# gpcv-liujin/Deep3D_Aerial

Hardware: AMD Instinct MI355X
Metric: cost-volume Mvoxels/s (5v x 384D) (higher is better)
Workload: dtype f32; 1 GPU; config 2: fused homography-warp + variance, 5 views x 384 planes, features 32x688x464 fp32 (2752x1856 image at 1/4 res), one reference view per step per GPU

## Files before the change

deep3d_aerial_amd/_lib.py:

```python
import ctypes
import os
import subprocess

_HERE = os.path.dirname(os.path.abspath(__file__))
CSRC = os.path.join(_HERE, "csrc")
SO_PATH = os.environ.get("D3D_LIBRARY") or os.path.join(CSRC, "libdeep3d_planesweep.so")
HEADER = os.path.join(os.path.dirname(_HERE), "include", "deep3d_planesweep.h")

ABI_VERSION = 11

_vp = ctypes.c_void_p
_i = ctypes.c_int
_i64 = ctypes.c_int64
_f = ctypes.c_float
_d = ctypes.c_double
_sz = ctypes.c_size_t

SIGNATURES = {
    "d3d_version": [],
    "d3d_last_error": ([], ctypes.c_char_p),
    "d3d_compose_projections": [_vp, _i, _vp, _vp],
    "d3d_debug_force_path": [_i],
    "d3d_debug_dispatch_counts": [_vp, _i],
    "d3d_build_flags": ([], ctypes.c_char_p),
    "d3d_h16_format": ([], ctypes.c_char_p),
    "d3d_compose_projections_f64": [_vp, _i, _vp, _vp],
    "d3d_homo_warp_f64coord": [_vp, _vp, _vp, _i, _i, _i, _i, _i, _vp, _vp],
    "d3d_sweep_workspace_bytes": ([_i, _i, _i, _i, _i, _i], _sz),
    "d3d_sweep_workspace_bytes_for": ([_i, _i, _i, _i, _i, _i, _i], _sz),
    "d3d_homo_warp": [_vp, _vp, _vp, _i, _i, _i, _i, _i, _vp, _vp, _sz, _vp],
    "d3d_variance_volume": [ctypes.POINTER(_vp), _vp, _vp, _i, _i, _i, _i, _i, _i, _vp, _vp, _sz, _vp],
    "d3d_variance_volume_planes": [ctypes.POINTER(_vp), _vp, _vp, _i, _i, _i, _i, _i, _i, _vp, _vp, _sz, _vp],
    "d3d_variance_volume_f16": [ctypes.POINTER(_vp), _vp, _vp, _i, _i, _i, _i, _i, _i, _vp, _vp, _sz, _vp],
    "d3d_variance_volume_cl_h16": [ctypes.POINTER(_vp), _vp, _vp, _i, _i, _i, _i, _i, _i, _vp, _vp, _sz, _vp],
    "d3d_variance_volume_cl8_h16": [ctypes.POINTER(_vp), _vp, _vp, _i, _i, _i, _i, _i, _i, _vp, _vp, _sz, _vp],
    "d3d_pair_corr_mean": [_vp, _vp, _vp, _vp, _i, _i, _i, _i, _i, _vp, _vp, _sz, _vp],
    "d3d_weighted_corr": [ctypes.POINTER(_vp), _vp, _vp, _vp, _i, _i, _i, _i, _i, _i, _i, _vp, _vp, _sz, _vp],
    "d3d_softargmin_conf4": [_vp, _vp, _i, _i, _i, _i, _vp, _vp, _vp],
    "d3d_online_regress_update": [_vp, _vp, _i, _i, _i, _i, _vp, _vp, _vp, _vp],
    "d3d_online_regress_finalize": [_vp, _vp, _vp, _i64, _vp, _vp, _vp],
    "d3d_depth_range_samples": [_vp, _i, _i, _f, _i, _i, _vp, _vp],
    "d3d_resize_bilinear": [_vp, _i, _i, _i, _i, _i, _vp, _vp],
    "d3d_conv3d_k3": [_vp, _vp, _vp, _vp, _vp, _i, _i, _i, _i, _i, _i, _i, _vp, _vp],
    "d3d_conv3d_k3_co8": [_vp, _vp, _vp, _vp, _vp, _i, _i, _i, _i, _i, _vp, _vp],
    "d3d_conv3d_k3_c8_h16": [_vp, _vp, _vp, _vp, _vp, _i, _i, _i, _i, _i, _vp, _vp],
    "d3d_conv3d_k3_zs_h16": [_vp, _vp, _vp, _vp, _vp, _i, _i, _i, _i, _i, _i, _vp, _vp],
    "d3d_conv3d_k3_zs_bf16x3": [_vp, _vp, _vp, _vp, _vp, _i, _i, _i, _i, _i, _i, _vp, _vp],
    "d3d_conv3d_k3_c1_bf16x3": [_vp, _vp, _vp, _vp, _vp, _i, _i, _i, _i, _i, _vp, _vp],
    "d3d_convtranspose3d_k3s2_zs_h16": [_vp, _vp, _vp, _vp, _vp, _i, _i, _i, _i, _i, _i, _vp, _vp],
    "d3d_convtranspose3d_k3s2_zs_bf16x3": [_vp, _vp, _vp, _vp, _vp, _i, _i, _i, _i, _i, _i, _vp, _vp],
    "d3d_conv2d_k3_zs_h16": [_vp, _i, _vp, _i, _vp, _vp, _vp, _vp, _vp, _i, _i, _i, _i, _i, _i, _vp, _vp],
    "d3d_conv2d_k3_zs_f32": [_vp, _i, _vp, _i, _vp, _vp, _vp, _vp, _vp, _i, _i, _i, _i, _i, _i, _vp, _vp],
    "d3d_conv2d_k3_zs_bf16x3": [_vp, _i, _vp, _i, _vp, _vp, _vp, _vp, _vp, _i, _i, _i, _i, _i, _i, _vp, _vp],
    "d3d_avgpool2d_4_8": [_vp, _i, _i, _i, _vp, _vp, _vp],
    "d3d_conv3x3_bias_border": [_vp, _vp, _i, _i, _i, _vp],
    "d3d_conv2d_k1_f32": [_vp, _vp, _vp, _vp, _vp, _i, _i, _i, _i, _i, _vp, _vp],
    "d3d_conv1x1_context": [_vp, _i, _vp, _vp, _i, _i, _vp, _i, _i, _i, _i, _i, _vp, _vp],
    "d3d_conv2d_k3s2_zs_h16": [_vp, _vp, _vp, _vp, _vp, _i, _i, _i, _i, _i, _i, _vp, _vp],
    "d3d_conv2d_k3s2_zs_h16_batched": [_vp, _vp, _vp, _vp, _i, _i, _i, _i, _i, _i, _i64, _i64, _vp, _vp],
    "d3d_conv2d_k3_wide_h16": [_vp, _i, _vp, _i, _vp, _vp, _vp, _vp, _i, _i, _i, _i, _vp, _vp],
    "d3d_slice_head_regress_h16": [_vp, _vp, _vp, _i, _vp, _i, _i, _i, _i, _vp, _vp, _vp, _vp],
    "d3d_gru_cell_fused_h16": [_vp, _i, _i, _i, _i, _vp, _i, _i, _i, _vp, _vp, _vp, _vp, _vp, _vp, _vp],
    "d3d_gru_cell_fused_cl8_h16": [_vp, _i, _vp, _i, _i, _i, _vp, _vp, _vp, _vp, _vp, _vp, _vp],
    "d3d_weighted_corr_cl8_h16": [ctypes.POINTER(_vp), _vp, _vp, _vp, _i, _i, _i, _i, _i, _i, _vp, _vp, _sz, _vp],
    "d3d_convtranspose2d_k3s2_zs_h16": [_vp, _vp, _vp, _vp, _vp, _i, _i, _i, _i, _i, _i, _vp, _vp],
    "d3d_conv2d_k3s2_zs_bf16x3": [_vp, _vp, _vp, _vp, _vp, _i, _i, _i, _i, _i, _i, _vp, _vp],
    "d3d_convtranspose2d_k3s2_zs_bf16x3": [_vp, _vp, _vp, _vp, _vp, _i, _i, _i, _i, _i, _i, _vp, _vp],
    "d3d_convtranspose2d_k4s2_zs_bf16x3": [_vp, _vp, _vp, _vp, _vp, _i, _i, _i, _i, _i, _i, _vp, _vp],
    "d3d_conv2d_k5s2_zs_bf16x3": [_vp, _vp, _vp, _vp, _vp, _i, _i, _i, _i, _i, _i, _vp, _vp],
    "d3d_conv2d_k3s2_zs_f32": [_vp, _vp, _vp, _vp, _vp, _i, _i, _i, _i, _i, _i, _vp, _vp],
    "d3d_convtranspose2d_k3s2_zs_f32": [_vp, _vp, _vp, _vp, _vp, _i, _i, _i, _i, _i, _i, _vp, _vp],
    "d3d_conv3d_k3_cl_h16": [_vp, _i, _vp, _vp, _vp, _vp, _i, _i, _i, _i, _i, _i, _vp, _i, _vp],
    "d3d_conv3d_k3_c1_cl_h16": [_vp, _i, _vp, _vp, _vp, _vp, _i, _i, _i, _i, _i, _vp, _vp],
    "d3d_conv3d_k3s2_cl_h16": [_vp, _vp, _vp, _vp, _vp, _i, _i, _i, _i, _i, _i, _vp, _vp],
    "d3d_convtranspose3d_k3s2_cl_h16": [_vp, _vp, _vp, _vp, _vp, _i, _i, _i, _i, _i, _i, _vp, _i, _vp],
    "d3d_conv2d_k3_zs_h16_gn": [_vp, _i, _vp, _i, _vp, _vp, _i, _i, _i, _vp, _vp, _i, _vp],
    "d3d_conv2d_k3_wide_h16_gn": [_vp, _i, _vp, _i, _vp, _vp, _i, _i, _i, _vp, _vp, _i, _vp],
    "d3d_convtranspose2d_k3s2_wide_h16": [_vp, _vp, _vp, _vp, _vp, _i, _i, _i, _i, _i, _vp, _vp],
    "d3d_conv2d_k3_pair3_bf16x3": [_vp, _vp, _vp, _vp, _i, _vp, _vp, _vp, _i, _i, _i, _i, _vp, _vp],
    "d3d_slice_tail_regress_h16": [_vp, _vp, _vp, _vp, _vp, _vp, _vp, _i, _i, _i, _i, _vp, _vp, _vp, _vp],
    "d3d_slice_tail_regress_same_h16": [_vp, _vp, _vp, _vp, _i, _vp, _vp, _vp, _i, _i, _i, _i, _vp, _vp, _vp, _vp],
    "d3d_conv3d_k3s2_zs_bf16x3": [_vp, _vp, _vp, _vp, _vp, _i, _i, _i, _i, _i, _i, _vp, _vp],
    "d3d_convtranspose3d_prob_cl_h16": [_vp, _vp, _vp, _vp, _vp, _i, _vp, _vp, _i, _i, _i, _vp, _vp],
    "d3d_volume_planar_to_cl_h16": [_vp, _i, _sz, _vp, _vp],
    "d3d_volume_cl_h16_to_planar": [_vp, _i, _sz, _vp, _vp],
    "d3d_convtranspose3d_k3s2_co8": [_vp, _vp, _vp, _vp, _vp, _i, _i, _i, _i, _i, _vp, _vp],
    "d3d_convtranspose3d_k3s2": [_vp, _vp, _vp, _vp, _vp, _i, _i, _i, _i, _i, _i, _vp, _vp],
    "d3d_conv1x1_upskip": [_vp, _i, _vp, _vp, _vp, _i, _i, _i, _vp, _vp],
    "d3d_conv2d_k3_stream": [_vp, _i, _vp, _i, _vp, _vp, _vp, _vp, _vp, _i, _i, _i, _i, _i, _vp, _vp],
    "d3d_conv2d_k3": [_vp, _i, _vp, _i, _vp, _vp, _vp, _vp, _i, _i, _i, _i, _i, _vp, _vp],
    "d3d_convtranspose2d_k3s2": [_vp, _vp, _vp, _vp, _vp, _i, _i, _i, _i, _i, _i, _vp, _vp],
    "d3d_conv_gemm_f32": [_vp, _i, _vp, _i, _vp, _i, _vp, _vp, _vp, _i, _i, _i, _i, _i, _i, _i, _i, _i, _i, _i, _i, _i,
                          _i, _i, _i, _i, _i, ctypes.c_char_p, _vp, _vp],
    "d3d_conv_fold_f32": [_vp, _i, _vp, _i, _vp, _i, _i, _vp, _vp, _vp, _i, _i, _vp, _i, _i, _i, _i, _i, _i, _i, _i,
                          ctypes.POINTER(ctypes.c_int), _i, ctypes.c_char_p, _vp, _vp],
    "d3d_conv_fold_h16": [_vp, _i, _vp, _i, _vp, _i, _i, _vp, _vp, _vp, _i, _i, _vp, _i, _i, _i, _i, _i, _i, _i, _i,
                           ctypes.POINTER(ctypes.c_int), _i, ctypes.c_char_p, _vp, _vp],
    "d3d_gru_gates": [_vp, _vp, _i, _i64, _vp, _vp, _vp],
    "d3d_gru_update": [_vp, _vp, _vp, _i64, _vp, _vp],
    "d3d_groupnorm_stats": [_vp, _i64, _i, _vp, _vp],
    "d3d_gru_gates_gn": [_vp, _vp, _vp, _vp, _vp, _vp, _vp, _vp, _i, _i64, ctypes.c_float, _i, _vp, _vp, _vp],
    "d3d_gru_update_gn": [_vp, _vp, _vp, _vp, _vp, _vp, _i, _i64, ctypes.c_float, _i, _vp, _vp],
    "d3d_gru_reset_gn": [_vp, _vp, _vp, _vp, _vp, _i, _i64, ctypes.c_float, _i, _vp, _vp],
    "d3d_gru_update_gates_gn": [_vp, _vp, _vp, _vp, _vp, _vp, _vp, _vp, _vp, _i, _i64, ctypes.c_float, _i, _vp, _vp],
    "d3d_gru2_cell_gn_h16": [_vp, _i, _vp, _i, _i, _i, _vp, _vp, _vp, _vp, _vp, _vp, _vp, _vp, _vp, _vp, ctypes.c_float, _i, _vp, _vp, _vp, _vp, _vp, _vp, _vp],
    "d3d_softargmin_conf4_var": [_vp, _vp, _i, _i, _i, _i, ctypes.c_float, _vp, _vp, _vp, _vp],
    "d3d_uncertainty_samples": [_vp, _vp, _i, _i, _i, _vp, _vp],
    "d3d_pair_softmax_max": [_vp, _vp, _i, _i, _i, _i, _vp, _vp, _vp],
    "d3d_consistency_check": [_vp, _vp, _vp, _vp, _vp, ctypes.POINTER(ctypes.c_double), _i, _i, _i, _i, ctypes.c_double,
                              _f, _f, _f, _vp, _vp, _vp, _vp, _vp, _vp],
    "d3d_fusion_ref_init": [_vp, _vp, ctypes.POINTER(ctypes.c_double), _i, _i, _vp, _vp, _vp, _vp, _vp],
    "d3d_fusion_accumulate": [_vp, _vp, _vp, _vp, _vp, ctypes.POINTER(ctypes.c_double), _i, _i, _i, _i,
                              ctypes.c_double, _f, _f, _f, _i, _vp, _vp, _vp, _vp, _vp, _vp],
    "d3d_fusion_finalize": [_vp, _vp, _vp, _i, _i, _i, _vp, _vp, _vp],
    "d3d_fusion_points_scratch_bytes": ([_i, _i], _sz),
    "d3d_fusion_mark_points": [_vp, _vp, _i, _i, _i, ctypes.POINTER(ctypes.c_double), _vp, _vp, _vp, _vp],
    "d3d_fusion_gather_points": [_vp, _vp, ctypes.POINTER(_vp), _i, _vp, _vp, _i, _i, _vp, _vp, _vp, _vp, _vp, _vp, _vp],
    "d3d_flip_rows": [ctypes.POINTER(_vp), _i, _i, _i, _vp, _vp],
    "d3d_center_image_u8": [_vp, _i, _i, _i, _i, _i, _i, _i, _i, _vp, _vp, _vp],
    "d3d_normals_from_depth": [_vp, ctypes.POINTER(_f), _i, _i, _i, _i, _vp, _vp, _vp],
    "d3d_dsm_scratch_bytes": ([ctypes.c_longlong, _i, _i, _i], _sz),
    "d3d_dsm_from_points": [_vp, ctypes.c_longlong, _d, _d, _d, _d, _d, _d, _i, _i, _i, _d, _i, _vp, _sz, _vp, _vp, _vp],
    "d3d_dsm_fill_moving_average": [_vp, _vp, _i, _i, _i, _vp],
    "d3d_dsm_mesh_scratch_bytes": ([ctypes.c_longlong, _i, _i], _sz),
    "d3d_dsm_from_mesh": [_vp, ctypes.c_longlong, _vp, ctypes.c_longlong, _d, _d, _d, _d, _d, _d, _i, _i, _vp, _sz, _vp, _vp],
    "d3d_ortho_scratch_bytes": ([_i, _i, _i], _sz),
    "d3d_ortho_select": [_vp, _d, _d, _d, _d, _i, _i, _vp, _i, _d, _vp, _sz, _vp, _vp],
    "d3d_ortho_colorize": [_vp, _d, _d, _d, _d, _i, _i, _vp, _vp, _i, _vp, _vp, _vp],
    "d3d_mesh_scan_scratch_bytes": ([ctypes.c_longlong], _sz),
    "d3d_mesh_mark": [_vp, _vp, _i, _i, _d, _vp, _vp],
    "d3d_mesh_bricks": [_vp, _vp, _vp, _sz, _vp, _vp, _vp, _vp],
    "d3d_mesh_integrate": [_vp, _vp, _i, _vp, _i, _d, _d, _vp, _vp, _vp],
    "d3d_mesh_count": [_vp, _vp, _vp, _i, _vp, _vp, _i, _vp, _sz, _vp, _vp, _vp, _vp, _vp],
    "d3d_mesh_emit": [_vp, _vp, _vp, _i, _vp, _vp, _i, _vp, _vp, _vp, _vp, _vp, _vp, _vp],
    "d3d_mesh_compact": [_vp, ctypes.c_longlong, _vp, ctypes.c_longlong, _vp, _vp, _sz, _vp, _vp, _vp, _vp],
    "d3d_mesh_adjacency_scratch_bytes": ([ctypes.c_longlong, ctypes.c_longlong], _sz),
    "d3d_mesh_adjacency": [_vp, ctypes.c_longlong, ctypes.c_longlong, _vp, _sz, _vp, _vp, _vp, _vp],
    "d3d_mesh_components": [_vp, ctypes.c_longlong, ctypes.c_longlong, _vp, _vp, ctypes.POINTER(_i), _vp],
    "d3d_mesh_stats_scratch_bytes": ([ctypes.c_longlong], _sz),
    "d3d_mesh_component_stats": [_vp, ctypes.c_longlong, _vp, ctypes.c_longlong, _vp, _vp, _sz, _vp, _vp, _vp, _vp, _vp, _vp],
    "d3d_mesh_filter_scratch_bytes": ([ctypes.c_longlong], _sz),
    "d3d_mesh_filter": [_vp, ctypes.c_longlong, ctypes.c_longlong, _vp, _vp, _vp, _vp, ctypes.c_longlong, _d, _vp, _sz, _vp, _vp, _vp, _vp],
    "d3d_mesh_smooth": [_vp, ctypes.c_longlong, _vp, _vp, _vp, _f, _i, _vp, _vp, _vp],
    "d3d_mesh_decimate_incidence_scratch_bytes": ([ctypes.c_longlong, ctypes.c_longlong], _sz),
    "d3d_mesh_decimate_incidence": [_vp, ctypes.c_longlong, ctypes.c_longlong, _vp, _sz, _vp, _vp, _vp],
    "d3d_mesh_decimate_quadrics": [_vp, ctypes.c_longlong, _vp, ctypes.c_longlong, _vp, _vp, _vp, _vp],
    "d3d_mesh_decimate_edges_scratch_bytes": ([ctypes.c_longlong], _sz),
    "d3d_mesh_decimate_edges": [_vp, _vp, ctypes.c_longlong, _vp, _sz, ctypes.c_longlong, _vp, _vp, _vp],
    "d3d_mesh_decimate_candidates": [_vp, ctypes.c_longlong, _vp, ctypes.c_longlong, _vp, _vp, _vp, _vp, _vp, _vp, _vp, _vp, ctypes.c_longlong, _vp, _vp, _vp, _vp],
    "d3d_mesh_decimate_select_scratch_bytes": ([], _sz),
    "d3d_mesh_decimate_select": [_vp, ctypes.c_longlong, ctypes.c_longlong, _vp, _sz, _vp, _vp],
    "d3d_mesh_decimate_claim": [_vp, _vp, ctypes.c_longlong, _vp, _vp, _vp, ctypes.c_longlong, _vp, _vp, _vp, _vp],
    "d3d_mesh_decimate_apply": [_vp, ctypes.c_longlong, _vp, _vp, _vp, _vp, _vp, _vp, _vp, ctypes.c_longlong, _vp, _vp, _vp, _vp, _vp, _vp, _vp],
    "d3d_mesh_decimate_faces_scratch_bytes": ([ctypes.c_longlong], _sz),
    "d3d_mesh_decimate_faces": [_vp, ctypes.c_longlong, ctypes.c_longlong, _vp, _vp, _sz, _vp, _vp, _vp, _vp],
    "d3d_mesh_holes_scratch_bytes": ([ctypes.c_longlong], _sz),
    "d3d_mesh_boundary": [_vp, ctypes.c_longlong, ctypes.c_longlong, _vp, _vp, _vp, _vp, _vp, _vp, _vp, _vp],
    "d3d_mesh_boundary_loops": [_vp, ctypes.c_longlong, ctypes.c_longlong, _vp, _vp, _vp, _vp, _vp, _vp, _vp, ctypes.POINTER(_i), _vp],
    "d3d_mesh_holes_plan": [_vp, ctypes.c_longlong, _vp, ctypes.c_longlong, _vp, _vp, _vp, _vp, _vp, _i, _vp, _sz, _vp, _vp, _vp, _vp, _vp, _vp,
                            _vp, _vp],
    "d3d_mesh_holes_emit": [_vp, ctypes.c_longlong, _vp, ctypes.c_longlong, _vp, _vp, _vp, _vp, _vp, _vp, _vp, ctypes.c_longlong,
                            ctypes.c_longlong, _vp, _vp, _vp],
    "d3d_texture_scratch_bytes": ([ctypes.c_longlong, _i], _sz),
    "d3d_texture_select": [_vp, ctypes.c_longlong, _vp, ctypes.c_longlong, _vp, _i, _d, _vp, _sz, _vp, _vp],
    "d3d_texture_edges": [_vp, ctypes.c_longlong, ctypes.c_longlong, _vp, _vp, _vp],
    "d3d_texture_charts": [_vp, _vp, ctypes.c_longlong, _vp, ctypes.c_longlong, _vp, _sz, _vp, _vp, _vp, _vp, ctypes.POINTER(_i), _vp],
    "d3d_texture_rects": [_vp, ctypes.c_longlong, _vp, ctypes.c_longlong, _vp, _vp, ctypes.c_longlong, _vp, _i, _i, _vp, _vp],
    "d3d_texture_fill": [_vp, ctypes.c_longlong, _vp, ctypes.c_longlong, _vp, _i, _vp, _i, _i, _vp, _vp],
    "d3d_texture_empty": [_vp, ctypes.c_longlong, ctypes.c_uint, _vp],
    "d3d_texture_texcoords": [_vp, ctypes.c_longlong, _vp, ctypes.c_longlong, _vp, _vp, _vp, ctypes.c_longlong, _vp, _i, _vp, _i, _i, _vp,
                              _vp, _vp],
}


class LibraryMissing(RuntimeError):
    pass


def build(verbose=False):
    cmd = ["make", "-C", CSRC, "-j4", "libdeep3d_planesweep.so"]
    res = subprocess.run(cmd, stdout=subprocess.PIPE, stderr=subprocess.STDOUT, text=True)
    if verbose or res.returncode != 0:
        print(res.stdout)
    if res.returncode != 0:
        raise RuntimeError("building libdeep3d_planesweep.so failed")
    return SO_PATH


_lib = None


def load():
    global _lib
    if _lib is not None:
        return _lib
    if not os.path.exists(SO_PATH):
        raise LibraryMissing(
            "%s not found -- build it with `python -c 'import __graft_entry__ as g; g.build()'` "
            "or `make -C deep3d_aerial_amd/csrc`. There is no CPU fallback." % SO_PATH)
    lib = ctypes.CDLL(SO_PATH)
    for name, sig in SIGNATURES.items():
        try:
            fn = getattr(lib, name)
        except AttributeError as e:
            raise LibraryMissing("symbol %s missing from %s" % (name, SO_PATH)) from e
        fn.argtypes, fn.restype = sig if isinstance(sig, tuple) else (sig, ctypes.c_int)
    if lib.d3d_version() != ABI_VERSION:
        raise LibraryMissing("ABI version mismatch: library %d, binding %d" % (lib.d3d_version(), ABI_VERSION))
    _lib = lib
    return lib


ERR_INVALID_ARG, ERR_UNSUPPORTED, ERR_HIP = -1, -2, -3


def h16_format():
    return load().d3d_h16_format().decode("ascii")


def code_objects(path=None):
    import struct

    data = open(path or SO_PATH, "rb").read()
    magic = b"__CLANG_OFFLOAD_BUNDLE__"
    pos = data.find(magic)
    while pos >= 0:
        n = struct.unpack_from("<Q", data, pos + 24)[0]
        q = pos + 32
        for _ in range(n):
            off, size, tl = struct.unpack_from("<QQQ", data, q)
            triple = data[q + 24:q + 24 + tl]
            q += 24 + tl
            if b"amdgcn" not in triple or size == 0:
                continue
            elf = data[pos + off:pos + off + size]
            if elf[:4] == b"\x7fELF":
                yield elf
        pos = data.find(magic, pos + len(magic))


def kernel_code_sha256(symbol_prefix, path=None):
    import hashlib
    import struct

    found = []
    for elf in code_objects(path):
        shoff, = struct.unpack_from("<Q", elf, 0x28)
        shentsize, shnum = struct.unpack_from("<HH", elf, 0x3A)
        secs = [struct.unpack_from("<IIQQQQIIQQ", elf, shoff + i * shentsize) for i in range(shnum)]
        for sh in secs:
            if sh[1] != 2:
                continue
            strtab = secs[sh[6]]
            for k in range(sh[5] // sh[9]):
                st_name, st_info, _, st_shndx, st_value, st_size = struct.unpack_from("<IBBHQQ", elf, sh[4] + k * sh[9])
                if (st_info & 0xF) != 2 or st_size == 0 or st_shndx >= len(secs):
                    continue
                end = elf.index(b"\0", strtab[4] + st_name)
                if elf[strtab[4] + st_name:end].decode("ascii", "replace").startswith(symbol_prefix):
                    sec = secs[st_shndx]
                    o = sec[4] + (st_value - sec[3])
                    found.append(hashlib.sha256(elf[o:o + st_size]).hexdigest())
    return found[0] if len(found) == 1 else None


def check(rc, what):
    if rc != 0:
        msg = load().d3d_last_error().decode("utf-8", "replace")
        kind = {-1: "invalid argument", -2: "unsupported", -3: "HIP error"}.get(rc, "error %d" % rc)
        raise RuntimeError("%s failed (%s): %s" % (what, kind, msg))
```

deep3d_aerial_amd/csrc/planesweep.hip:

```cpp
#include <hip/hip_fp16.h>

#include "common.h"

#include <array>
#include <atomic>
#include <cstring>
#include <mutex>
#include <unordered_map>

namespace d3d {

static thread_local char g_err[512] = "";

void set_error(const char* fmt, ...) {
    va_list ap;
    va_start(ap, fmt);
    vsnprintf(g_err, sizeof(g_err), fmt, ap);
    va_end(ap);
}

int hip_status(hipError_t e, const char* what) {
    if (e == hipSuccess) return D3D_OK;
    set_error("%s: %s", what, hipGetErrorString(e));
    return D3D_ERR_HIP;
}

int ensure_dynamic_lds(const void* kernel, int bytes) {
    constexpr int MAXDEV = 16;
    static std::mutex mu;
    static std::unordered_map<const void*, std::array<int, MAXDEV>> granted;
    int dev = 0;
    if (hipGetDevice(&dev) != hipSuccess) dev = -1;
    if (dev >= 0 && dev < MAXDEV) {
        std::lock_guard<std::mutex> lock(mu);
        auto it = granted.find(kernel);
        if (it != granted.end() && it->second[dev] >= bytes) return D3D_OK;
    }
    const int rc = hip_status(hipFuncSetAttribute(kernel, hipFuncAttributeMaxDynamicSharedMemorySize, bytes),
                              "hipFuncSetAttribute(MaxDynamicSharedMemorySize)");
    if (rc == D3D_OK && dev >= 0 && dev < MAXDEV) {
        std::lock_guard<std::mutex> lock(mu);
        auto& slot = granted[kernel];
        if (slot[dev] < bytes) slot[dev] = bytes;
    }
    return rc;
}

int launch_tiled(int mode, const struct SweepParams& p, hipStream_t stream);
int launch_window(int mode, const struct SweepParams& p, hipStream_t stream, bool forced);
size_t tiled_workspace_bytes(int n_src, int C, int D, int h, int w, int elem_bytes);
size_t window_workspace_bytes(int n_src, int C, int D, int h, int w, int elem_bytes);
const char* tiled_build_flags();
const char* window_build_flags();
const char* gru_build_flags();

}

#include "sweep_params.h"

namespace d3d {

__global__ void compose_kernel(const float* __restrict__ proj44, int n_views, float* __restrict__ out34) {
    int i = blockIdx.x * blockDim.x + threadIdx.x + 1;
    if (i >= n_views) return;
    double m[16], inv[16];
    for (int k = 0; k < 16; ++k) m[k] = (double)proj44[k];
    inv[0] = m[5] * m[10] * m[15] - m[5] * m[11] * m[14] - m[9] * m[6] * m[15] + m[9] * m[7] * m[14] +
             m[13] * m[6] * m[11] - m[13] * m[7] * m[10];
    inv[4] = -m[4] * m[10] * m[15] + m[4] * m[11] * m[14] + m[8] * m[6] * m[15] - m[8] * m[7] * m[14] -
             m[12] * m[6] * m[11] + m[12] * m[7] * m[10];
    inv[8] = m[4] * m[9] * m[15] - m[4] * m[11] * m[13] - m[8] * m[5] * m[15] + m[8] * m[7] * m[13] +
             m[12] * m[5] * m[11] - m[12] * m[7] * m[9];
    inv[12] = -m[4] * m[9] * m[14] + m[4] * m[10] * m[13] + m[8] * m[5] * m[14] - m[8] * m[6] * m[13] -
              m[12] * m[5] * m[10] + m[12] * m[6] * m[9];
    inv[1] = -m[1] * m[10] * m[15] + m[1] * m[11] * m[14] + m[9] * m[2] * m[15] - m[9] * m[3] * m[14] -
             m[13] * m[2] * m[11] + m[13] * m[3] * m[10];
    inv[5] = m[0] * m[10] * m[15] - m[0] * m[11] * m[14] - m[8] * m[2] * m[15] + m[8] * m[3] * m[14] +
             m[12] * m[2] * m[11] - m[12] * m[3] * m[10];
    inv[9] = -m[0] * m[9] * m[15] + m[0] * m[11] * m[13] + m[8] * m[1] * m[15] - m[8] * m[3] * m[13] -
             m[12] * m[1] * m[11] + m[12] * m[3] * m[9];
    inv[13] = m[0] * m[9] * m[14] - m[0] * m[10] * m[13] - m[8] * m[1] * m[14] + m[8] * m[2] * m[13] +
              m[12] * m[1] * m[10] - m[12] * m[2] * m[9];
    inv[2] = m[1] * m[6] * m[15] - m[1] * m[7] * m[14] - m[5] * m[2] * m[15] + m[5] * m[3] * m[14] +
             m[13] * m[2] * m[7] - m[13] * m[3] * m[6];
    inv[6] = -m[0] * m[6] * m[15] + m[0] * m[7] * m[14] + m[4] * m[2] * m[15] - m[4] * m[3] * m[14] -
             m[12] * m[2] * m[7] + m[12] * m[3] * m[6];
    inv[10] = m[0] * m[5] * m[15] - m[0] * m[7] * m[13] - m[4] * m[1] * m[15] + m[4] * m[3] * m[13] +
              m[12] * m[1] * m[7] - m[12] * m[3] * m[5];
    inv[14] = -m[0] * m[5] * m[14] + m[0] * m[6] * m[13] + m[4] * m[1] * m[14] - m[4] * m[2] * m[13] -
              m[12] * m[1] * m[6] + m[12] * m[2] * m[5];
    inv[3] = -m[1] * m[6] * m[11] + m[1] * m[7] * m[10] + m[5] * m[2] * m[11] - m[5] * m[3] * m[10] -
             m[9] * m[2] * m[7] + m[9] * m[3] * m[6];
    inv[7] = m[0] * m[6] * m[11] - m[0] * m[7] * m[10] - m[4] * m[2] * m[11] + m[4] * m[3] * m[10] +
             m[8] * m[2] * m[7] - m[8] * m[3] * m[6];
    inv[11] = -m[0] * m[5] * m[11] + m[0] * m[7] * m[9] + m[4] * m[1] * m[11] - m[4] * m[3] * m[9] -
              m[8] * m[1] * m[7] + m[8] * m[3] * m[5];
    inv[15] = m[0] * m[5] * m[10] - m[0] * m[6] * m[9] - m[4] * m[1] * m[10] + m[4] * m[2] * m[9] +
              m[8] * m[1] * m[6] - m[8] * m[2] * m[5];
    double det = m[0] * inv[0] + m[1] * inv[4] + m[2] * inv[8] + m[3] * inv[12];
    double idet = 1.0 / det;
    const float* s = proj44 + 16 * i;
    for (int r = 0; r < 3; ++r)
        for (int c = 0; c < 4; ++c) {
            double acc = 0.0;
            for (int k = 0; k < 4; ++k) acc += (double)s[r * 4 + k] * (inv[k * 4 + c] * idet);
            out34[(i - 1) * 12 + r * 4 + c] = (float)acc;
        }
}

struct TapD {
    int off;
    int dx, dyw;
    float nw, ne, sw, se;
};

__device__ __forceinline__ TapD make_tap_direct(float u, float v, int h, int w) {
    TapD t;
    float fu = floorf(u), fv = floorf(v);
    int x0 = (int)fu, y0 = (int)fv;
    float ax = u - fu, ay = v - fv;
    float bx = (fu + 1.0f) - u, by = (fv + 1.0f) - v;
    bool vx0 = (x0 >= 0) && (x0 < w), vx1 = (x0 >= -1) && (x0 < w - 1);
    bool vy0 = (y0 >= 0) && (y0 < h), vy1 = (y0 >= -1) && (y0 < h - 1);
    t.nw = (vx0 && vy0) ? bx * by : 0.0f;
    t.ne = (vx1 && vy0) ? ax * by : 0.0f;
    t.sw = (vx0 && vy1) ? bx * ay : 0.0f;
    t.se = (vx1 && vy1) ? ax * ay : 0.0f;
    int x0c = min(max(x0, 0), w - 1), x1c = min(max(x0 + 1, 0), w - 1);
    int y0c = min(max(y0, 0), h - 1), y1c = min(max(y0 + 1, 0), h - 1);
    t.off = y0c * w + x0c;
    t.dx = x1c - x0c;
    t.dyw = (y1c - y0c) * w;
    return t;
}

__device__ __forceinline__ float ldf(const float* p) { return *p; }
__device__ __forceinline__ float ldf(const __half* p) { return __half2float(*p); }
__device__ __forceinline__ void stf(float* p, float v) { *p = v; }
__device__ __forceinline__ void stf(__half* p, float v) {
    *p = __float2half_rn(sat_f16(v));
}

template <typename T>
__device__ __forceinline__ float gather4(const T* __restrict__ f, const TapD& t) {
    const T* q = f + t.off;
    float acc = ldf(q) * t.nw;
    acc = fmaf(ldf(q + t.dx), t.ne, acc);
    acc = fmaf(ldf(q + t.dyw), t.sw, acc);
    acc = fmaf(ldf(q + t.dyw + t.dx), t.se, acc);
    return acc;
}

template <int MODE, int CC, typename T = float>
__global__ __launch_bounds__(256) void sweep_direct_kernel(SweepParams p) {
    const int x = blockIdx.x * 64 + (threadIdx.x & 63);
    const int y = blockIdx.y * 4 + (threadIdx.x >> 6);
    if (x >= p.w || y >= p.h) return;
    const int h = p.h, w = p.w, C = p.C, D = p.D;
    const size_t plane = (size_t)h * w;
    const size_t pix = (size_t)y * w + x;
    const float xf = (float)x, yf = (float)y;
    const int d0 = blockIdx.z * p.d_chunk;
    const int d1 = min(d0 + p.d_chunk, D);
    const float invV = 1.0f / (float)(p.n_src + 1);

    for (int d = d0; d < d1; ++d) {
        const float dv = p.depth_mode == D3D_DEPTH_PER_PIXEL ? p.depth[(size_t)d * plane + pix]
                         : p.depth_mode == D3D_DEPTH_AFFINE ? __fadd_rn(p.depth[pix], __fmul_rn((float)d, p.depth[plane + pix]))
                                                            : p.depth[d];
        float den = 1e-5f;
        if (MODE == MODE_WEIGHTED)
            for (int i = 0; i < p.n_src; ++i) den += p.weights[(size_t)i * plane + pix];
        float pair_acc = 0.0f;
        for (int c0 = 0; c0 < C; c0 += CC) {
            float s[CC], q[CC], r[CC];
#pragma unroll
            for (int c = 0; c < CC; ++c) {
                r[c] = (MODE == MODE_WARP) ? 0.0f : ldf(reinterpret_cast<const T*>(p.feats[0]) + (size_t)(c0 + c) * plane + pix);
                s[c] = (MODE == MODE_VARIANCE) ? r[c] : 0.0f;
                q[c] = r[c] * r[c];
            }
            for (int i = 0; i < p.n_src; ++i) {
                const float* __restrict__ P = p.proj34 + 12 * i;
                Ray ray = make_ray(P, xf, yf);
                float u, v;
                project(ray, P[3], P[7], P[11], dv, h, w, u, v);
                TapD t = make_tap_direct(u, v, h, w);
                const T* __restrict__ f = reinterpret_cast<const T*>(p.feats[i + 1]) + (size_t)c0 * plane;
                float vw = (MODE == MODE_WEIGHTED) ? p.weights[(size_t)i * plane + pix] : 0.0f;
#pragma unroll
                for (int c = 0; c < CC; ++c) {
                    float val = gather4(f + (size_t)c * plane, t);
                    if (MODE == MODE_VARIANCE) {
                        s[c] += val;
                        q[c] = fmaf(val, val, q[c]);
                    } else if (MODE == MODE_WEIGHTED) {
                        s[c] = fmaf(val * r[c], vw, s[c]);
                    } else if (MODE == MODE_PAIR) {
                        pair_acc = fmaf(r[c], val, pair_acc);
                    } else {
                        s[c] = val;
                    }
                }
            }
            if (MODE != MODE_PAIR) {
#pragma unroll
                for (int c = 0; c < CC; ++c) {
                    float o;
                    if (MODE == MODE_VARIANCE) {
                        float m = s[c] * invV;
                        o = fmaf(q[c], invV, -(m * m));
                    } else if (MODE == MODE_WEIGHTED) {
                        o = s[c] / den;
                    } else {
                        o = s[c];
                    }
                    stf(reinterpret_cast<T*>(p.out) + (p.plane_major ? (size_t)d * C + (c0 + c) : (size_t)(c0 + c) * D + d) * plane + pix, o);
                }
            }
        }
        if (MODE == MODE_PAIR) stf(reinterpret_cast<T*>(p.out) + (size_t)d * plane + pix, pair_acc / (float)C);
    }
}


__global__ void compose_f64_kernel(const double* __restrict__ proj44, int n_views, double* __restrict__ out34) {
    int i = blockIdx.x * blockDim.x + threadIdx.x + 1;
    if (i >= n_views) return;
    double a[4][8];
    for (int r = 0; r < 4; ++r)
        for (int c = 0; c < 4; ++c) { a[r][c] = proj44[r * 4 + c]; a[r][4 + c] = r == c ? 1.0 : 0.0; }
    for (int col = 0; col < 4; ++col) {
        int piv = col;
        for (int r = col + 1; r < 4; ++r) if (fabs(a[r][col]) > fabs(a[piv][col])) piv = r;
        for (int c = 0; c < 8; ++c) { double t = a[col][c]; a[col][c] = a[piv][c]; a[piv][c] = t; }
        const double inv = 1.0 / a[col][col];
        for (int c = 0; c < 8; ++c) a[col][c] *= inv;
        for (int r = 0; r < 4; ++r) {
            if (r == col) continue;
            const double f = a[r][col];
            for (int c = 0; c < 8; ++c) a[r][c] -= f * a[col][c];
        }
    }
    const double* s = proj44 + 16 * i;
    for (int r = 0; r < 3; ++r)
        for (int c = 0; c < 4; ++c) {
            double acc = 0.0;
            for (int k = 0; k < 4; ++k) acc += s[r * 4 + k] * a[k][4 + c];
            out34[(i - 1) * 12 + r * 4 + c] = acc;
        }
}

__global__ __launch_bounds__(256) void warp_f64coord_kernel(const float* __restrict__ src, const double* __restrict__ P,
                                                            const float* __restrict__ depth, int depth_mode, int C, int D,
                                                            int h, int w, float* __restrict__ out) {
    const int x = blockIdx.x * 64 + (threadIdx.x & 63);
    const int y = blockIdx.y * 4 + (threadIdx.x >> 6);
    const int d = blockIdx.z;
    if (x >= w || y >= h) return;
    const size_t plane = (size_t)h * w, pix = (size_t)y * w + x;
    const double dv = (double)(depth_mode == D3D_DEPTH_PER_PIXEL ? depth[(size_t)d * plane + pix] : depth[d]);
    const double xd = (double)x, yd = (double)y;
    const double rx = P[0] * xd + P[1] * yd + P[2];
    const double ry = P[4] * xd + P[5] * yd + P[6];
    const double rz = P[8] * xd + P[9] * yd + P[10];
    const double px = rx * dv + P[3], py = ry * dv + P[7], pz = rz * dv + P[11];
    const float gx = (float)((px / pz) / ((double)(w - 1) / 2.0) - 1.0);
    const float gy = (float)((py / pz) / ((double)(h - 1) / 2.0) - 1.0);
    const float ix = ((gx + 1.0f) / 2.0f) * (float)(w - 1);
    const float iy = ((gy + 1.0f) / 2.0f) * (float)(h - 1);
    const bool ok = (ix > -2.0f) && (ix < (float)w + 1.0f) && (iy > -2.0f) && (iy < (float)h + 1.0f);
    const TapD t = make_tap_direct(ok ? ix : -2.0f, ok ? iy : -2.0f, h, w);
    for (int c = 0; c < C; ++c)
        out[((size_t)c * D + d) * plane + pix] = gather4(src + (size_t)c * plane, t);
}

template <int MODE, typename T = float>
static int launch_direct(const SweepParams& p, hipStream_t stream) {
    SweepParams q = p;
    q.d_chunk = 8;
    dim3 grid(ceil_div(p.w, 64), ceil_div(p.h, 4), ceil_div(p.D, q.d_chunk));
    dim3 block(256);
    if (p.C % 16 == 0)
        hipLaunchKernelGGL((sweep_direct_kernel<MODE, 16, T>), grid, block, 0, stream, q);
    else if (p.C % 8 == 0)
        hipLaunchKernelGGL((sweep_direct_kernel<MODE, 8, T>), grid, block, 0, stream, q);
    else if (p.C % 4 == 0)
        hipLaunchKernelGGL((sweep_direct_kernel<MODE, 4, T>), grid, block, 0, stream, q);
    else
        hipLaunchKernelGGL((sweep_direct_kernel<MODE, 1, T>), grid, block, 0, stream, q);
    D3D_LAUNCH_CHECK("sweep_direct_kernel launch");
    return D3D_OK;
}

static int check_dims(int C, int D, int h, int w) {
    D3D_REQUIRE(C > 0 && D > 0 && h > 1 && w > 1, "bad dims C=%d D=%d h=%d w=%d (need C,D>0 and h,w>1)", C, D, h, w);
    D3D_REQUIRE((long)h * w < (1L << 30), "feature map too large: %d x %d", h, w);
    D3D_REQUIRE(ceil_div(h, 4) <= 65535 && ceil_div(D, 8) <= 65535, "grid too large (h=%d D=%d)", h, D);
    return D3D_OK;
}

static std::atomic<int> g_force_path{0};
static int forced_path() { return g_force_path.load(std::memory_order_relaxed); }

static std::atomic<unsigned long long> g_dispatched[4];
static int counted(int family, int rc) {
    if (rc == D3D_OK) g_dispatched[family].fetch_add(1, std::memory_order_relaxed);
    return rc;
}

static int sweep_dispatch(int mode, const SweepParams& p, hipStream_t stream) {
    const int force = forced_path();
    if (force == 0 || force == 3) {
        int rc = counted(3, launch_window(mode, p, stream, force == 3));
        if (rc != D3D_ERR_UNSUPPORTED || force == 3) return rc;
    }
    if (force != 1) {
        int rc = counted(2, launch_tiled(mode, p, stream));
        if (rc != D3D_ERR_UNSUPPORTED) return rc;
        if (force == 2) return rc;
    }
    if (p.elem_bytes == 2) return counted(1, launch_direct<MODE_VARIANCE, __half>(p, stream));
    switch (mode) {
        case MODE_WARP: return counted(1, launch_direct<MODE_WARP>(p, stream));
        case MODE_VARIANCE: return counted(1, launch_direct<MODE_VARIANCE>(p, stream));
        case MODE_WEIGHTED: return counted(1, launch_direct<MODE_WEIGHTED>(p, stream));
        case MODE_PAIR: return counted(1, launch_direct<MODE_PAIR>(p, stream));
    }
    set_error("internal: bad mode %d", mode);
    return D3D_ERR_INVALID_ARG;
}

}

using namespace d3d;

extern "C" {

int d3d_version(void) { return D3D_ABI_VERSION; }

const char* d3d_last_error(void) { return g_err; }

int d3d_compose_projections(const float* proj44, int n_views, float* out34, d3d_stream_t stream) {
    D3D_REQUIRE(proj44 && out34, "null pointer");
    D3D_REQUIRE(n_views >= 2 && n_views <= D3D_MAX_VIEWS, "n_views=%d out of range [2,%d]", n_views, D3D_MAX_VIEWS);
    hipLaunchKernelGGL(compose_kernel, dim3(1), dim3(64), 0, (hipStream_t)stream, proj44, n_views, out34);
    D3D_LAUNCH_CHECK("compose_kernel launch");
    return D3D_OK;
}

int d3d_debug_dispatch_counts(unsigned long long* out4, int reset) {
    D3D_REQUIRE(out4, "null pointer");
    for (int i = 0; i < 4; ++i) out4[i] = reset ? g_dispatched[i].exchange(0, std::memory_order_relaxed) : g_dispatched[i].load(std::memory_order_relaxed);
    return D3D_OK;
}

const char* d3d_h16_format(void) { return D3D_H16_FORMAT; }

const char* d3d_build_flags(void) {
    static char buf[512];
    static std::atomic<int> done{0};
    if (!done.load(std::memory_order_acquire)) {
        char tmp[512];
        snprintf(tmp, sizeof(tmp), "%s%s%s", tiled_build_flags(), window_build_flags(), gru_build_flags());
        const char* s = tmp;
        while (*s == ' ') ++s;
        snprintf(buf, sizeof(buf), "%s", s);
        done.store(1, std::memory_order_release);
    }
    return buf;
}

int d3d_debug_force_path(int path) {
    D3D_REQUIRE(path >= 0 && path <= 3, "path must be 0 (auto), 1 (direct), 2 (tiled) or 3 (window)");
    g_force_path.store(path, std::memory_order_relaxed);
    return D3D_OK;
}

size_t d3d_sweep_workspace_bytes_for(int n_views, int C, int D, int h, int w, int elem_bytes, int depth_mode) {
    if (n_views < 2 || C <= 0 || D <= 0 || h <= 1 || w <= 1 || (elem_bytes != 4 && elem_bytes != 2)) return 0;
    const size_t a = tiled_workspace_bytes(n_views - 1, C, D, h, w, elem_bytes);
    const size_t b = depth_mode == D3D_DEPTH_PER_PIXEL ? window_workspace_bytes(n_views - 1, C, D, h, w, elem_bytes) : 0;
    return a > b ? a : b;
}

size_t d3d_sweep_workspace_bytes(int n_views, int C, int D, int h, int w, int elem_bytes) {
    return d3d_sweep_workspace_bytes_for(n_views, C, D, h, w, elem_bytes, D3D_DEPTH_PER_PIXEL);
}

int d3d_homo_warp(const float* src, const float* proj34, const float* depth, int depth_mode, int C, int D, int h,
                  int w, float* out, void* workspace, size_t workspace_bytes, d3d_stream_t stream) {
    D3D_REQUIRE(src && proj34 && depth && out, "null pointer");
    D3D_REQUIRE(depth_mode == 0 || depth_mode == 1, "bad depth_mode %d", depth_mode);
    int rc = check_dims(C, D, h, w);
    if (rc) return rc;
    SweepParams p = {};
    p.feats[0] = src;
    p.feats[1] = src;
    p.proj34 = proj34;
    p.depth = depth;
    p.out = out;
    p.n_src = 1;
    p.C = C; p.D = D; p.h = h; p.w = w;
    p.depth_mode = depth_mode;
    p.elem_bytes = 4;
    p.workspace = workspace;
    p.workspace_bytes = workspace ? workspace_bytes : 0;
    return sweep_dispatch(MODE_WARP, p, (hipStream_t)stream);
}

int d3d_compose_projections_f64(const double* proj44, int n_views, double* out34, d3d_stream_t stream) {
    D3D_REQUIRE(proj44 && out34, "null pointer");
    D3D_REQUIRE(n_views >= 2 && n_views <= D3D_MAX_VIEWS, "n_views=%d out of range [2,%d]", n_views, D3D_MAX_VIEWS);
    hipLaunchKernelGGL(compose_f64_kernel, dim3(1), dim3(64), 0, (hipStream_t)stream, proj44, n_views, out34);
    D3D_LAUNCH_CHECK("compose_f64_kernel launch");
    return D3D_OK;
}

int d3d_homo_warp_f64coord(const float* src, const double* proj34, const float* depth, int depth_mode, int C, int D,
                           int h, int w, float* out, d3d_stream_t stream) {
    D3D_REQUIRE(src && proj34 && depth && out, "null pointer");
    D3D_REQUIRE(depth_mode == 0 || depth_mode == 1, "bad depth_mode %d", depth_mode);
    int rc = check_dims(C, D, h, w);
    if (rc) return rc;
    D3D_REQUIRE(D <= 65535, "D=%d too large for one launch", D);
    hipLaunchKernelGGL(warp_f64coord_kernel, dim3(ceil_div(w, 64), ceil_div(h, 4), D), dim3(256), 0, (hipStream_t)stream, src,
                       proj34, depth, depth_mode, C, D, h, w, out);
    D3D_LAUNCH_CHECK("warp_f64coord_kernel launch");
    return D3D_OK;
}

static int fill_multi(SweepParams& p, const float* const* feats, const float* proj34, const float* depth,
                      int depth_mode, int n_views, int C, int D, int h, int w, float* out, void* workspace,
                      size_t workspace_bytes, int elem_bytes = 4) {
    D3D_REQUIRE(feats && proj34 && depth && out, "null pointer");
    D3D_REQUIRE(n_views >= 2 && n_views <= D3D_MAX_VIEWS, "n_views=%d out of range [2,%d]", n_views, D3D_MAX_VIEWS);
    D3D_REQUIRE(depth_mode >= 0 && depth_mode <= 2, "bad depth_mode %d", depth_mode);
    int rc = check_dims(C, D, h, w);
    if (rc) return rc;
    for (int i = 0; i < n_views; ++i) {
        D3D_REQUIRE(feats[i], "feats[%d] is null", i);
        p.feats[i] = feats[i];
    }
    p.proj34 = proj34;
    p.depth = depth;
    p.out = out;
    p.n_src = n_views - 1;
    p.C = C; p.D = D; p.h = h; p.w = w;
    p.depth_mode = depth_mode;
    p.elem_bytes = elem_bytes;
    p.workspace = workspace;
    p.workspace_bytes = workspace ? workspace_bytes : 0;
    return D3D_OK;
}

int d3d_variance_volume(const float* const* feats, const float* proj34, const float* depth, int depth_mode,
                        int n_views, int C, int D, int h, int w, float* out, void* workspace, size_t workspace_bytes,
                        d3d_stream_t stream) {
    SweepParams p = {};
    int rc = fill_multi(p, feats, proj34, depth, depth_mode, n_views, C, D, h, w, out, workspace, workspace_bytes);
    if (rc) return rc;
    return sweep_dispatch(MODE_VARIANCE, p, (hipStream_t)stream);
}

int d3d_variance_volume_planes(const float* const* feats, const float* proj34, const float* depth, int depth_mode,
                               int n_views, int C, int D, int h, int w, float* out, void* workspace, size_t workspace_bytes,
                               d3d_stream_t stream) {
    SweepParams p = {};
    int rc = fill_multi(p, feats, proj34, depth, depth_mode, n_views, C, D, h, w, out, workspace, workspace_bytes);
    if (rc) return rc;
    p.plane_major = 1;
    return sweep_dispatch(MODE_VARIANCE, p, (hipStream_t)stream);
}

static int variance_volume_cl_any(int layout, const float* const* feats, const float* proj34, const float* depth, int depth_mode,
                                int n_views, int C, int D, int h, int w, void* out, void* workspace, size_t workspace_bytes,
                                d3d_stream_t stream) {
    SweepParams p = {};
    int rc = fill_multi(p, feats, proj34, depth, depth_mode, n_views, C, D, h, w, reinterpret_cast<float*>(out), workspace,
                        workspace_bytes);
    if (rc) return rc;
    p.out_cl = layout;
    if (forced_path() == 1) {
        set_error("d3d_variance_volume_cl_h16: only the LDS-ring and window kernels write channel-last volumes");
        return D3D_ERR_UNSUPPORTED;
    }
    if (forced_path() != 2) {
        rc = counted(3, launch_window(MODE_VARIANCE, p, (hipStream_t)stream, forced_path() == 3));
        if (rc != D3D_ERR_UNSUPPORTED || forced_path() == 3) return rc;
    }
    return counted(2, launch_tiled(MODE_VARIANCE, p, (hipStream_t)stream));
}

int d3d_variance_volume_cl_h16(const float* const* feats, const float* proj34, const float* depth, int depth_mode,
                                int n_views, int C, int D, int h, int w, void* out, void* workspace, size_t workspace_bytes,
                                d3d_stream_t stream) {
    return variance_volume_cl_any(1, feats, proj34, depth, depth_mode, n_views, C, D, h, w, out, workspace, workspace_bytes, stream);
}

int d3d_variance_volume_cl8_h16(const float* const* feats, const float* proj34, const float* depth, int depth_mode,
                                 int n_views, int C, int D, int h, int w, void* out, void* workspace, size_t workspace_bytes,
                                 d3d_stream_t stream) {
    return variance_volume_cl_any(2, feats, proj34, depth, depth_mode, n_views, C, D, h, w, out, workspace, workspace_bytes, stream);
}

int d3d_variance_volume_f16(const void* const* feats, const float* proj34, const float* depth, int depth_mode,
                            int n_views, int C, int D, int h, int w, void* out, void* workspace, size_t workspace_bytes,
                            d3d_stream_t stream) {
    SweepParams p = {};
    int rc = fill_multi(p, reinterpret_cast<const float* const*>(feats), proj34, depth, depth_mode, n_views, C, D, h, w,
                        reinterpret_cast<float*>(out), workspace, workspace_bytes, 2);
    if (rc) return rc;
    return sweep_dispatch(MODE_VARIANCE, p, (hipStream_t)stream);
}

int d3d_weighted_corr(const float* const* feats, const float* proj34, const float* weights, const float* depth,
                      int depth_mode, int n_views, int C, int D, int h, int w, int plane_major, float* out, void* workspace,
                      size_t workspace_bytes, d3d_stream_t stream) {
    SweepParams p = {};
    D3D_REQUIRE(weights, "null weights");
    D3D_REQUIRE(plane_major == 0 || plane_major == 1, "bad plane_major %d", plane_major);
    int rc = fill_multi(p, feats, proj34, depth, depth_mode, n_views, C, D, h, w, out, workspace, workspace_bytes);
    if (rc) return rc;
    p.weights = weights;
    p.plane_major = plane_major;
    return sweep_dispatch(MODE_WEIGHTED, p, (hipStream_t)stream);
}

int d3d_weighted_corr_cl8_h16(const float* const* feats, const float* proj34, const float* weights, const float* depth,
                              int depth_mode, int n_views, int C, int D, int h, int w, void* out, void* workspace,
                              size_t workspace_bytes, d3d_stream_t stream) {
    SweepParams p = {};
    D3D_REQUIRE(weights, "null weights");
    int rc = fill_multi(p, feats, proj34, depth, depth_mode, n_views, C, D, h, w, reinterpret_cast<float*>(out), workspace, workspace_bytes);
    if (rc) return rc;
    p.weights = weights;
    p.out_cl = 2;
    if (forced_path() == 1 || forced_path() == 2) {
        set_error("d3d_weighted_corr_cl8_h16: only the window kernel writes the channel-last correlation volume");
        return D3D_ERR_UNSUPPORTED;
    }
    return counted(3, launch_window(MODE_WEIGHTED, p, (hipStream_t)stream, forced_path() == 3));
}

int d3d_pair_corr_mean(const float* ref, const float* src, const float* proj34, const float* depth, int depth_mode,
                       int C, int D, int h, int w, float* out, void* workspace, size_t workspace_bytes,
                       d3d_stream_t stream) {
    const float* feats[2] = {ref, src};
    SweepParams p = {};
    int rc = fill_multi(p, feats, proj34, depth, depth_mode, 2, C, D, h, w, out, workspace, workspace_bytes);
    if (rc) return rc;
    return sweep_dispatch(MODE_PAIR, p, (hipStream_t)stream);
}

}
```

deep3d_aerial_amd/csrc/planesweep_tiled.hip:

```cpp
#include "common.h"

#include <hip/hip_fp16.h>

#include "sweep_params.h"
#include "sweep_device.h"

#include <cstdlib>

namespace d3d {

namespace {

constexpr int TW = 32;
constexpr int TH = 4;
constexpr int NPIXW = 2;
#ifndef D3D_NSUB
#define D3D_NSUB 4
#endif
#ifndef D3D_NLOADW
#define D3D_NLOADW 4
#endif
constexpr int NSUB = D3D_NSUB;
constexpr int NCOMP = NPIXW * NSUB;
constexpr int NLOADW = D3D_NLOADW;
constexpr int NWAVES = NCOMP + NLOADW;
constexpr int THREADS = 64 * NWAVES;
constexpr int DSEG_MAX = 128;
constexpr int MAXSTEPS = 64;
constexpr int PFD = 2;
#ifndef D3D_LDS_PIPE
#define D3D_LDS_PIPE 1
#endif
#ifndef D3D_GRAB
#define D3D_GRAB 0
#endif
#ifndef D3D_FREERUN
#define D3D_FREERUN 0
#endif
constexpr int LDS_PIPE = D3D_LDS_PIPE;
constexpr int NCAND = 4;
constexpr int MAXRECTS = 512;
constexpr int RING_RW_QUANT = 8;
constexpr int RING_RH_QUANT = 2;
template <int STRIDE>
__host__ __device__ __forceinline__ int ring_row_floats(int RW) {
    const int n = (RW + 1) * STRIDE;
    return ((n - 32 + 63) & ~63) + 32;
}

#ifdef D3D_EXPERIMENTS
#define D3D_STAMPS 1
#else
#define D3D_STAMPS 0
#endif
#define D3D_CLOCK() (D3D_STAMPS ? clock64() : 0ll)

struct TiledArgs {
    int ngroups;
    int dseg;
    int cap_floats;
    int nseg;
    int tiles_x, tiles_y;
    const float* cl;
    unsigned long long* tstats;
    unsigned* stats;
};

template <int CW, int NSRC>
struct Lds {
    static constexpr int STRIDE = CW + 4;
    static constexpr int ZERO = 0;
    static constexpr int PMIN = 2 * STRIDE;
    static constexpr int PMAX = PMIN + DSEG_MAX;
    static constexpr int HDR = PMAX + DSEG_MAX;
    static constexpr int VT = HDR + 32;
    static constexpr int CNT = VT + 8 * NSRC;
    static constexpr int PLAN = CNT + 2 * MAXSTEPS;
    static constexpr int SST = PLAN + MAXSTEPS * NSRC * 8;
    static constexpr int STOT = SST + MAXSTEPS + 4;
    static constexpr int RECTS = ((STOT + MAXSTEPS + 3) / 4) * 4;
    static constexpr int DATA = RECTS + (MAXRECTS + 1) * 4;
};

struct Rects {
    int rx[4], ry[4], rw[4], rh[4], start[5];
};


#ifndef D3D_DECOUPLE
#define D3D_DECOUPLE 0
#endif
#ifndef STAGE0_ALL
#define STAGE0_ALL 1
#endif
#define STAGE0_ALL_EFF (STAGE0_ALL && !D3D_DECOUPLE)
__device__ __forceinline__ void step_signal(int* ctr, int lane) {
    __builtin_amdgcn_fence(__ATOMIC_RELEASE, "workgroup");
    if (lane == 0) __hip_atomic_fetch_add(ctr, 1, __ATOMIC_RELAXED, __HIP_MEMORY_SCOPE_WORKGROUP);
}
__device__ __forceinline__ void step_wait(int* ctr, int target) {
#ifndef D3D_SPIN_LOG2
#define D3D_SPIN_LOG2 16
#endif
    for (int spin = 0; spin < (1 << D3D_SPIN_LOG2); ++spin) {
        if (__hip_atomic_load(ctr, __ATOMIC_RELAXED, __HIP_MEMORY_SCOPE_WORKGROUP) >= target) break;
        __builtin_amdgcn_s_sleep(2);
    }
    __builtin_amdgcn_fence(__ATOMIC_ACQUIRE, "workgroup");
}
__device__ __forceinline__ void ctr_add(int* ctr, int lane) {
    asm volatile("" ::: "memory");
    if (lane == 0) __hip_atomic_fetch_add(ctr, 1, __ATOMIC_RELAXED, __HIP_MEMORY_SCOPE_WORKGROUP);
    asm volatile("" ::: "memory");
}
__device__ __forceinline__ void ctr_wait(int* ctr, int target) {
    for (int spin = 0; spin < (1 << 22); ++spin) {
        const int v = __builtin_amdgcn_readfirstlane(__hip_atomic_load(ctr, __ATOMIC_RELAXED, __HIP_MEMORY_SCOPE_WORKGROUP));
        if (v >= target) break;
        __builtin_amdgcn_s_sleep(1);
    }
    asm volatile("" ::: "memory");
}
__device__ __forceinline__ int posmod(int a, int n) {
    int r = a % n;
    return r < 0 ? r + n : r;
}


struct RingView {
    int RW, RH;
    int rowb;
    int base;
};

template <int STRIDE>
__device__ __forceinline__ TapL geo_ring(const Ray& r, float tx, float ty, float tz, float d, float umax, float vmax, int kx, int ky,
                                         const RingView& R) {
    const float px = __fadd_rn(__fmul_rn(r.rx, d), tx);
    const float py = __fadd_rn(__fmul_rn(r.ry, d), ty);
    const float pz = __fadd_rn(__fmul_rn(r.rz, d), tz);
    const float iz = __builtin_amdgcn_rcpf(pz);
    const float u0 = px * iz, v0 = py * iz;
    float u = fmaf(fmaf(-u0, pz, px), iz, u0);
    float v = fmaf(fmaf(-v0, pz, py), iz, v0);
    u = __builtin_amdgcn_fmed3f(u, -1.0f, umax);
    v = __builtin_amdgcn_fmed3f(v, -1.0f, vmax);
    const float fu = floorf(u), fv = floorf(v);
    const float ax = u - fu, ay = v - fv;
    const float bx = (fu + 1.0f) - u, by = (fv + 1.0f) - v;
    TapL t;
    t.nw = bx * by;
    t.ne = ax * by;
    t.sw = bx * ay;
    t.se = ax * ay;
    unsigned c = (unsigned)((int)fu + kx), rr = (unsigned)((int)fv + ky);
    c = min(c, c - (unsigned)R.RW);
    rr = min(rr, rr - (unsigned)R.RH);
    t.a0 = R.base + (int)__umul24(rr, (unsigned)R.rowb) + (int)__umul24(c, (unsigned)(STRIDE * 4));
    t.a1 = t.a0 + R.rowb;
    return t;
}


__device__ __forceinline__ void store_sbase_h(unsigned long long sb, unsigned byte_off, float v) {
    const _Float16 hv = (_Float16)sat_f16(v);
    const unsigned bits = __builtin_bit_cast(unsigned short, hv);
    asm volatile("global_store_short %0, %1, %2 nt" : : "v"(byte_off), "v"(bits), "s"(sb));
}
typedef _Float16 h8 __attribute__((ext_vector_type(8)));
__device__ __forceinline__ float fma_mix_lo(float pair, float w, float acc) {
    float d;
    asm("v_fma_mix_f32 %0, %1, %2, %3 op_sel_hi:[1,0,0]" : "=v"(d) : "v"(pair), "v"(w), "v"(acc));
    return d;
}
__device__ __forceinline__ float fma_mix_hi(float pair, float w, float acc) {
    float d;
    asm("v_fma_mix_f32 %0, %1, %2, %3 op_sel:[1,0,0] op_sel_hi:[1,0,0]" : "=v"(d) : "v"(pair), "v"(w), "v"(acc));
    return d;
}
__device__ __forceinline__ float ldf(const float* q) { return *q; }
__device__ __forceinline__ float ldf(const __half* q) { return __half2float(*q); }

}

template <int MODE, int NSRC, int CH, typename T = float, bool OUTCL = false, int NSUB_T = D3D_NSUB, int NLOAD_T = D3D_NLOADW,
          int NPIXW_T = 2>
__global__ __launch_bounds__(64 * (NPIXW_T * NSUB_T + NLOAD_T), 3) void sweep_tiled_kernel(SweepParams p, TiledArgs a) {
    constexpr int NSUB = NSUB_T, NLOADW = NLOAD_T, NPIXW = NPIXW_T, TH = 2 * NPIXW;
    constexpr int NCOMP = NPIXW * NSUB, NWAVES = NCOMP + NLOADW, THREADS = 64 * NWAVES;
    constexpr bool F16 = sizeof(T) == 2;
    static_assert(!OUTCL || (MODE == MODE_VARIANCE && !F16), "channel-last bf16 output is built for the fp32 variance volume");
    constexpr int CW = CH * (int)sizeof(T) / 4;
    constexpr int CPC = 16 / (int)sizeof(T);
    using L = Lds<CW, NSRC>;
    constexpr int STRIDE = L::STRIDE;
    constexpr int Q = CW / 4;
    static_assert(!F16 || MODE == MODE_VARIANCE, "fp16 storage is built for the variance volume only");
    constexpr bool VIEW_MAJOR = F16;
    constexpr bool FREERUN = D3D_FREERUN && NLOADW > 0 && NPIXW <= 2;
    constexpr int MAXRS = 4 * NSRC;
    static_assert(NSRC <= 15, "rect descriptors keep the view in 4 bits");
    extern __shared__ __attribute__((aligned(16))) float lds[];
    int* ldsi = reinterpret_cast<int*>(lds);

    const long long t_start = D3D_CLOCK();
    const int tid = threadIdx.x;
    const int lane = tid & 63;
    const int wave = rfl(tid >> 6);
    const bool loader = wave >= NCOMP;
    const int lw = wave - NCOMP;
    const int pw = (wave % NCOMP) % NPIXW;
    const int sub = (wave % NCOMP) / NPIXW;
    const int h = p.h, w = p.w, D = p.D;
    const size_t plane = (size_t)h * w;

    int b = blockIdx.x;
    {
        const int nblk = gridDim.x;
        const int per = nblk / 8;
        if (nblk % 8 == 0) b = (b % 8) * per + b / 8;
    }
    const int ty = b % a.tiles_y;
    const int seg = (b / a.tiles_y) % a.nseg;
    const int tx = b / (a.tiles_y * a.nseg);
    const int x0 = tx * TW, y0 = ty * TH;
    const int ds = seg * a.dseg;
    const int de = min(ds + a.dseg, D);
    const int nplanes = de - ds;
    const int x1c = min(x0 + TW - 1, w - 1), y1c = min(y0 + TH - 1, h - 1);

    const int l5 = lane & 31;
    const int pxl = (l5 < 4) ? l5 : (l5 < 12) ? l5 + 4 : (l5 < 20) ? l5 - 8 : (l5 < 28) ? l5 - 20 : l5 - 16;
    const int px = x0 + pxl + 16 * (lane >> 5);
    const int py = y0 + pw * 2 + (l5 >> 4);
    const bool valid = (px < w) && (py < h);
    const int pix = valid ? py * w + px : 0;
    const unsigned pixb = (unsigned)pix * (unsigned)sizeof(T);
    const unsigned pixo = OUTCL ? (p.out_cl == 2 ? (unsigned)pix * 16u : (unsigned)pix * (unsigned)p.C * 2u) : pixb;
    const float xf = (float)px, yf = (float)py;

    constexpr bool EARLY_INPUTS = NSRC <= 4 && !F16 && CH <= 16;
    int grp = 0, c0 = 0;
    Ray ray[NSRC];
    float T0[NSRC], T1[NSRC], T2[NSRC];
    auto projection_rows = [&]() {
#pragma unroll
        for (int i = 0; i < NSRC; ++i) {
            const float* __restrict__ M = p.proj34 + 12 * min(i, p.n_src - 1);
            ray[i] = make_ray(M, xf, yf);
            T0[i] = M[3]; T1[i] = M[7]; T2[i] = M[11];
            if constexpr (EARLY_INPUTS) asm volatile("" : "+v"(T0[i]), "+v"(T1[i]), "+v"(T2[i]));
        }
    };
    if constexpr (EARLY_INPUTS) projection_rows();
    f4 r[F16 ? 1 : Q];
    float rh[F16 ? Q : 1][8];
    auto load_reference = [&]() {
        if (F16) {
#pragma unroll
            for (int q = 0; q < Q; ++q)
#pragma unroll
                for (int k = 0; k < 8; ++k) {
                    float t = ldf(reinterpret_cast<const T*>(p.feats[0]) + (size_t)(c0 + 8 * q + k) * plane + pix);
                    rh[F16 ? q : 0][k] = valid ? t : 0.0f;
                }
        } else if (MODE != MODE_WARP) {
#pragma unroll
            for (int q = 0; q < Q; ++q)
#pragma unroll
                for (int k = 0; k < 4; ++k) {
                    float t = p.feats[0][(size_t)(c0 + 4 * q + k) * plane + pix];
                    r[F16 ? 0 : q][k] = valid ? t : 0.0f;
                }
        }
    };
    float vw[NSRC];
    float rden = 0.0f;
    float aff_lo = 1.0f, aff_step = 0.0f;
    auto lane_inputs = [&]() {
        if (MODE == MODE_WEIGHTED) {
            float den = 1e-5f;
#pragma unroll
            for (int i = 0; i < NSRC; ++i) {
                float t = p.weights[(size_t)min(i, p.n_src - 1) * plane + pix];
                vw[i] = (valid && i < p.n_src) ? t : 0.0f;
                den += vw[i];
            }
            rden = 1.0f / den;
        }
        load_reference();
        if (p.depth_mode == D3D_DEPTH_AFFINE && valid) {
            aff_lo = p.depth[pix];
            aff_step = p.depth[plane + pix];
        }
    };
    if (EARLY_INPUTS && !loader) lane_inputs();

    for (int i = tid; i < 2 * STRIDE; i += THREADS) lds[L::ZERO + i] = 0.0f;
    if (p.depth_mode == D3D_DEPTH_PER_PLANE) {
        for (int i = tid; i < nplanes; i += THREADS) {
            float dv = p.depth[ds + i];
            lds[L::PMIN + i] = dv;
            lds[L::PMAX + i] = dv;
        }
    } else if (p.depth_mode == D3D_DEPTH_AFFINE) {
        float blo[(TW * TH) / 64], bst[(TW * TH) / 64];
        bool bok[(TW * TH) / 64];
#pragma unroll
        for (int k = 0; k < (TW * TH) / 64; ++k) {
            const int q = lane + 64 * k;
            const int qx = x0 + (q & 31), qy = y0 + (q >> 5);
            bok[k] = qx < w && qy < h;
            const size_t qi = bok[k] ? (size_t)qy * w + qx : 0;
            blo[k] = p.depth[qi];
            bst[k] = p.depth[plane + qi];
        }
        for (int i = wave; i < nplanes; i += NWAVES) {
            float lo = INFINITY, hi = -INFINITY;
#pragma unroll
            for (int k = 0; k < (TW * TH) / 64; ++k) {
                const float dv = __fadd_rn(blo[k], __fmul_rn((float)(ds + i), bst[k]));
                if (bok[k]) { lo = fminf(lo, dv); hi = fmaxf(hi, dv); }
            }
            lo = wave_min(lo);
            hi = wave_max(hi);
            if (lane == 0) {
                lds[L::PMIN + i] = lo;
                lds[L::PMAX + i] = hi;
            }
        }
    } else {
        for (int i = wave; i < nplanes; i += NWAVES) {
            float lo = INFINITY, hi = -INFINITY;
#pragma unroll
            for (int k = 0; k < (TW * TH) / 64; ++k) {
                int q = lane + 64 * k;
                int qx = x0 + (q & 31), qy = y0 + (q >> 5);
                if (qx < w && qy < h) {
                    float dv = p.depth[(size_t)(ds + i) * plane + (size_t)qy * w + qx];
                    lo = fminf(lo, dv);
                    hi = fmaxf(hi, dv);
                }
            }
            lo = wave_min(lo);
            hi = wave_max(hi);
            if (lane == 0) {
                lds[L::PMIN + i] = lo;
                lds[L::PMAX + i] = hi;
            }
        }
    }
    __syncthreads();
    const long long t_range = D3D_CLOCK();

    constexpr int CT = L::DATA;
    constexpr int CHD = CT + NCAND * NSRC * 64 * 4;
    auto cand_planes = [](int c) { return c < 3 ? NSUB * (4 >> c) : max(NSUB / 2, 1); };
    auto candidate_windows = [&](int cand, int vsel) {
        {
            const int SPc = cand_planes(cand);
            const int nstepc = (nplanes + SPc - 1) / SPc;
            const bool feasible = nstepc <= MAXSTEPS;
            const bool act = feasible && lane < nstepc;
            const int p0 = min(lane * SPc, nplanes - 1), p1 = min(lane * SPc + SPc, nplanes);
            float lo = INFINITY, hi = -INFINITY;
            for (int i = p0; i < p1; ++i) {
                lo = fminf(lo, lds[L::PMIN + i]);
                hi = fmaxf(hi, lds[L::PMAX + i]);
            }
            const float* __restrict__ M = p.proj34 + 12 * min(vsel, p.n_src - 1);
            float umin = INFINITY, umax = -INFINITY, vmin = INFINITY, vmax = -INFINITY;
            bool ok = true;
#pragma unroll
            for (int ck = 0; ck < 8; ++ck) {
                Ray cr = make_ray(M, (ck & 1) ? (float)x1c : (float)x0, (ck & 2) ? (float)y1c : (float)y0);
                const float dv = (ck & 4) ? hi : lo;
                float qx = __fadd_rn(__fmul_rn(cr.rx, dv), M[3]);
                float qy = __fadd_rn(__fmul_rn(cr.ry, dv), M[7]);
                float qz = __fadd_rn(__fmul_rn(cr.rz, dv), M[11]);
                ok = ok && (qz > 1e-20f) && (qz < 1e30f);
                float iz = 1.0f / qz;
                float u = qx * iz, v = qy * iz;
                ok = ok && (fabsf(u) < 1e30f) && (fabsf(v) < 1e30f);
                u = fminf(fmaxf(u, -1.0f), (float)w);
                v = fminf(fmaxf(v, -1.0f), (float)h);
                umin = fminf(umin, u); umax = fmaxf(umax, u);
                vmin = fminf(vmin, v); vmax = fmaxf(vmax, v);
            }
            int wx0 = max((int)floorf(umin - 0.0625f), -1);
            int wy0 = max((int)floorf(vmin - 0.0625f), -1);
            int wx1 = min((int)floorf(umax + 0.0625f) + 1, w + 1);
            int wy1 = min((int)floorf(vmax + 0.0625f) + 1, h + 1);
            int ww = max(wx1 - wx0 + 1, 0), wh = max(wy1 - wy0 + 1, 0);
            if (vsel >= p.n_src) { wx0 = -1; wy0 = -1; ww = 2; wh = 2; ok = true; }
            if (!act) { ww = 0; wh = 0; ok = true; }
            int ux = ww, uy = wh;
            {
                const int qx0 = __shfl_up(wx0, 1), qy0 = __shfl_up(wy0, 1);
                const int qw = __shfl_up(ww, 1), qh = __shfl_up(wh, 1);
                if (lane > 0 && act && qw > 0 && ww > 0) {
                    ux = max(wx0 + ww, qx0 + qw) - min(wx0, qx0);
                    uy = max(wy0 + wh, qy0 + qh) - min(wy0, qy0);
                }
            }
            const int RWc = max(wave_maxi(ux), 1), RHc = max(wave_maxi(uy), 1);
            const int badc = (__any(!ok) || !feasible) ? 1 : 0;
            int* e = ldsi + CT + ((cand * NSRC + vsel) * 64 + lane) * 4;
            e[0] = wx0; e[1] = wy0; e[2] = ww; e[3] = wh;
            if (lane == 0) {
                int* hd = ldsi + CHD + (cand * NSRC + vsel) * 4;
                hd[0] = RWc; hd[1] = RHc; hd[2] = badc; hd[3] = nstepc;
            }
        }
    };
    constexpr int NCAND1 = NCAND - 1;
    for (int wk = wave; wk < NCAND1 * NSRC; wk += NWAVES) candidate_windows(wk / NSRC, wk % NSRC);
    __syncthreads();
    const long long t_p1 = D3D_CLOCK();
    auto plan_tables = [&](int cbeg, int cend) {
        int mode = 0, sp_sel = NSUB, nsteps_sel = (nplanes + NSUB - 1) / NSUB;
        for (int cand = cbeg; cand < cend && !mode; ++cand) {
            const int nsteps = ldsi[CHD + (cand * NSRC) * 4 + 3];
            const bool act = lane < nsteps;
            int wx0[NSRC], wy0[NSRC], ww[NSRC], wh[NSRC], RW[NSRC], RH[NSRC];
            int bad = 0, total = 0, totalq = 0;
            int RWq[NSRC], RHq[NSRC];
#pragma unroll
            for (int i = 0; i < NSRC; ++i) {
                const int* hd = ldsi + CHD + (cand * NSRC + i) * 4;
                RW[i] = hd[0]; RH[i] = hd[1]; bad |= hd[2];
                RWq[i] = (RW[i] + RING_RW_QUANT - 1) / RING_RW_QUANT * RING_RW_QUANT;
                RHq[i] = (RH[i] + RING_RH_QUANT - 1) / RING_RH_QUANT * RING_RH_QUANT;
                total += ring_row_floats<STRIDE>(RW[i]) * (RH[i] + 1);
                totalq += ring_row_floats<STRIDE>(RWq[i]) * (RHq[i] + 1);
            }
            if (totalq <= a.cap_floats) {
                total = totalq;
#pragma unroll
                for (int i = 0; i < NSRC; ++i) { RW[i] = RWq[i]; RH[i] = RHq[i]; }
            }
            if (bad || total > a.cap_floats) continue;
#pragma unroll
            for (int i = 0; i < NSRC; ++i) {
                const int* e = ldsi + CT + ((cand * NSRC + i) * 64 + lane) * 4;
                wx0[i] = e[0]; wy0[i] = e[1]; ww[i] = e[2]; wh[i] = e[3];
            }
            if (!bad && total <= a.cap_floats) {
                mode = 1;
                sp_sel = cand_planes(cand);
                nsteps_sel = nsteps;
                int base = L::DATA;
                int oxv[NSRC], oyv[NSRC], basev[NSRC];
                bool dims_ok = true;
#pragma unroll
                for (int i = 0; i < NSRC; ++i) {
                    const int cx0 = __shfl(wx0[i], 0), cy0 = __shfl(wy0[i], 0);
                    oxv[i] = posmod(wx0[i] - cx0, RW[i]);
                    oyv[i] = posmod(wy0[i] - cy0, RH[i]);
                    basev[i] = base;
                    dims_ok = dims_ok && RW[i] < 256 && RH[i] < 256;
                    if (act) {
                        int* e = ldsi + L::PLAN + (lane * NSRC + i) * 8;
                        e[0] = wx0[i]; e[1] = wy0[i]; e[2] = ww[i]; e[3] = wh[i];
                        e[4] = oxv[i];
                        e[5] = oyv[i];
                        e[6] = oxv[i] - wx0[i];
                        e[7] = oyv[i] - wy0[i];
                    }
                    if (lane == 0) {
                        ldsi[L::HDR + 4 + 4 * i + 0] = RW[i];
                        ldsi[L::HDR + 4 + 4 * i + 1] = RH[i];
                        ldsi[L::HDR + 4 + 4 * i + 2] = base;
                        ldsi[L::HDR + 4 + 4 * i + 3] = RW[i] | (RH[i] << 8) | ((base >> 2) << 16);
                        if constexpr (VIEW_MAJOR) {
                            const float* __restrict__ M = p.proj34 + 12 * min(i, p.n_src - 1);
                            const bool dummy = i >= p.n_src;
                            lds[L::VT + 8 * i + 0] = dummy ? -1.0f : M[3];
                            lds[L::VT + 8 * i + 1] = dummy ? -1.0f : M[7];
                            lds[L::VT + 8 * i + 2] = dummy ? 1.0f : M[11];
                            lds[L::VT + 8 * i + 3] = 0.0f;
                            ldsi[L::VT + 8 * i + 4] = RW[i];
                            ldsi[L::VT + 8 * i + 5] = RH[i];
                            ldsi[L::VT + 8 * i + 6] = ring_row_floats<STRIDE>(RW[i]) * 4;
                            ldsi[L::VT + 8 * i + 7] = lds_base_bytes(lds) + 4 * base;
                        }
                    }
                    base += ring_row_floats<STRIDE>(RW[i]) * (RH[i] + 1);
                }
                int cnt[NSRC][4], rx[NSRC][4], ry[NSRC][4], rwid[NSRC][4], nel[NSRC][4];
                int npos = 0;
#pragma unroll
                for (int i = 0; i < NSRC; ++i) {
                    const int xa = wx0[i], xb = wx0[i] + ww[i] - 1, ya = wy0[i], yb = wy0[i] + wh[i] - 1;
                    const int pxa = __shfl_up(wx0[i], 1), pya = __shfl_up(wy0[i], 1);
                    const int pxb = pxa + __shfl_up(ww[i], 1) - 1, pyb = pya + __shfl_up(wh[i], 1) - 1;
                    int ix0 = 1, ix1 = 0, iy0 = 1, iy1 = 0;
                    if (lane > 0) { ix0 = max(xa, pxa); ix1 = min(xb, pxb); iy0 = max(ya, pya); iy1 = min(yb, pyb); }
                    const bool ov = (ix0 <= ix1) && (iy0 <= iy1);
                    int rh_[4];
                    rx[i][0] = xa;      ry[i][0] = ya;      rwid[i][0] = (ov ? ix0 - 1 : xb) - xa + 1; rh_[0] = wh[i];
                    rx[i][1] = ix1 + 1; ry[i][1] = ya;      rwid[i][1] = ov ? xb - ix1 : 0;             rh_[1] = wh[i];
                    rx[i][2] = ix0;     ry[i][2] = ya;      rwid[i][2] = ov ? ix1 - ix0 + 1 : 0;        rh_[2] = ov ? iy0 - ya : 0;
                    rx[i][3] = ix0;     ry[i][3] = iy1 + 1; rwid[i][3] = ov ? ix1 - ix0 + 1 : 0;        rh_[3] = ov ? yb - iy1 : 0;
#pragma unroll
                    for (int r = 0; r < 4; ++r) {
                        nel[i][r] = act ? max(rwid[i][r], 0) * max(rh_[r], 0) : 0;
                        cnt[i][r] = (nel[i][r] + 63) >> 6;
                        npos += nel[i][r];
                    }
                }
                int nrect = 0;
#pragma unroll
                for (int i = 0; i < NSRC; ++i)
#pragma unroll
                    for (int r = 0; r < 4; ++r) nrect += cnt[i][r] > 0 ? 1 : 0;
                int incl = nrect;
#pragma unroll
                for (int sft = 1; sft < 64; sft <<= 1) {
                    int o = __shfl_up(incl, sft);
                    if (lane >= sft) incl += o;
                }
                const int total_rects = __shfl(incl, 63);
                if (total_rects > MAXRECTS || !dims_ok || __any(npos > 0xffff) || w > 0xfff0 || h > 0xfff0) {
                    mode = 0;
                } else {
                    int idx = incl - nrect;
                    if (act) ldsi[L::SST + lane] = idx;
                    if (lane == nsteps - 1) ldsi[L::SST + nsteps] = incl;
                    int pstart = 0;
#pragma unroll
                    for (int i = 0; i < NSRC; ++i)
#pragma unroll
                        for (int r = 0; r < 4; ++r)
                            if (cnt[i][r] > 0) {
                                int* e = ldsi + L::RECTS + 4 * idx;
                                e[0] = (rx[i][r] + 1) | ((ry[i][r] + 1) << 16);
                                e[1] = rwid[i][r] | (i << 12) | (pstart << 16);
                                e[2] = nel[i][r];
                                e[3] = (rx[i][r] - wx0[i] + oxv[i]) | ((ry[i][r] - wy0[i] + oyv[i]) << 16);
                                pstart += nel[i][r];
                                ++idx;
                            }
                    if (act) ldsi[L::STOT + lane] = pstart;
                }
            }
        }
        if (lane == 0) {
            ldsi[L::HDR + 0] = mode;
            ldsi[L::HDR + 1] = sp_sel;
            ldsi[L::HDR + 2] = nsteps_sel;
        }
        for (int i = lane; i < 2 * MAXSTEPS; i += 64) ldsi[L::CNT + i] = 0;
        if (lane < 2) ldsi[L::HDR + 28 + lane] = 0;
    };
    if (wave == 0) plan_tables(0, NCAND1);
    __syncthreads();
    if (rfl(ldsi[L::HDR + 0]) == 0) {
        __syncthreads();
        for (int wk = wave; wk < NSRC; wk += NWAVES) candidate_windows(NCAND1, wk);
        __syncthreads();
        if (wave == 0) plan_tables(NCAND1, NCAND);
        __syncthreads();
    }
    if (D3D_STAMPS && a.tstats && tid == 0) {
        const long long t_p2 = clock64();
        atomicAdd(a.tstats + 16, (unsigned long long)(t_range - t_start));
        atomicAdd(a.tstats + 17, (unsigned long long)(t_p1 - t_range));
        atomicAdd(a.tstats + 18, (unsigned long long)(t_p2 - t_p1));
    }
    const int ring = rfl(ldsi[L::HDR + 0]);
    const int SP = rfl(ldsi[L::HDR + 1]);
    const int nsteps = rfl(ldsi[L::HDR + 2]);
    if (D3D_STAMPS && a.stats && tid == 0) {
        atomicAdd(a.stats + (ring ? 0 : 1), 1u);
        atomicAdd(a.stats + 2, (unsigned)SP);
        atomicAdd(a.stats + 3, (unsigned)nsteps);
        if (ring) {
            unsigned tot = 0;
            for (int i = 0; i < NSRC; ++i) tot += (ldsi[L::HDR + 4 + 4 * i] + 1) * (ldsi[L::HDR + 5 + 4 * i] + 1);
            atomicAdd(a.stats + 4, tot);
        }
    }
    struct Item {
        const float* g;
        int meta;
        int geo;
    };
    long long fdelta[NSRC];
#pragma unroll
    for (int i = 0; i < NSRC; ++i) {
        const long long d0 = reinterpret_cast<long long>(p.feats[1]);
        const long long di = reinterpret_cast<long long>(p.feats[i + 1]);
        fdelta[i] = (i < p.n_src) ? di - d0 : 0;
    }
    auto item = [&](int el, int Tn, int rb, const int (&pst16)[MAXRS]) -> Item {
        Item I;
        const bool live = el < Tn;
        int ridx = rb - 1;
#pragma unroll
        for (int rr = 0; rr < MAXRS; ++rr) ridx += (pst16[rr] <= el) ? 1 : 0;
        ridx = max(ridx, rb);
        const int* e = ldsi + L::RECTS + 4 * ridx;
        const int e0 = e[0], e1 = e[1], e6 = e[3];
        const int rx = (e0 & 0xffff) - 1, ry = (e0 >> 16) - 1;
        const int rwid = e1 & 0xfff, vi = (e1 >> 12) & 0xf, pst = (unsigned)e1 >> 16;
        const int e7 = ldsi[L::HDR + 4 + 4 * vi + 3];
        const int RWv = e7 & 0xff, RHv = (e7 >> 8) & 0xff, bs = (e7 >> 16) << 2;
        const int pos = el - pst;
        const int cy = (int)(((float)pos + 0.5f) * __builtin_amdgcn_rcpf((float)max(rwid, 1)));
        const int cx = pos - cy * rwid;
        const int sx = rx + cx, sy = ry + cy;
        const bool ok = live && ((unsigned)sx < (unsigned)w) && ((unsigned)sy < (unsigned)h);
        long long dsel = 0;
#pragma unroll
        for (int i = 1; i < NSRC; ++i) dsel = (vi == i) ? fdelta[i] : dsel;
        if (a.cl)
            I.g = a.cl + ((size_t)(vi * a.ngroups + grp) * plane + (size_t)(ok ? sy * w + sx : 0)) * CW;
        else
            I.g = reinterpret_cast<const float*>(reinterpret_cast<const char*>(p.feats[1]) + dsel) + (size_t)c0 * plane +
                  (ok ? sy * w + sx : 0);
        unsigned c = (unsigned)((e6 & 0xffff) + cx), r = (unsigned)((e6 >> 16) + cy);
        c = min(c, c - (unsigned)RWv);
        r = min(r, r - (unsigned)RHv);
        const int dst = bs + (int)r * ring_row_floats<STRIDE>(RWv) + (int)c * STRIDE;
        I.meta = live ? (dst | (ok ? 1 << 20 : 0) | (c == 0 ? 1 << 21 : 0) | (r == 0 ? 1 << 22 : 0)) : -1;
        I.geo = e7 & 0xffff;
        return I;
    };
    auto put = [&](int meta, int geo, int q, f4 v) {
        if (meta >= 0) {
            const int dst = (meta & 0xfffff) + 4 * q;
            const int RWv = geo & 0xff, RHv = geo >> 8;
            const int dupc = (meta >> 21) & 1 ? RWv * STRIDE : 0;
            const int dupr = (meta >> 22) & 1 ? RHv * ring_row_floats<STRIDE>(RWv) : 0;
            f4 x = (meta >> 20) & 1 ? v : (f4){0, 0, 0, 0};
            *reinterpret_cast<f4*>(lds + dst) = x;
            if (dupc) *reinterpret_cast<f4*>(lds + dst + dupc) = x;
            if (dupr) *reinterpret_cast<f4*>(lds + dst + dupr) = x;
            if (dupc && dupr) *reinterpret_cast<f4*>(lds + dst + dupc + dupr) = x;
        }
    };
    f4 pf[PFD][Q];
    int pmeta[PFD], pgeo[PFD];
    auto write_round = [&]() {
#pragma unroll
        for (int j = 0; j < PFD; ++j)
#pragma unroll
            for (int q = 0; q < Q; ++q) put(pmeta[j], pgeo[j], q, pf[j][q]);
    };
    const bool ltiming = D3D_STAMPS && a.tstats != nullptr && lw == 0;
    long long lt_desc = 0, lt_issue = 0, lt_write = 0, lt_bar = 0;
    auto stage = [&](int k, int sw, int snw) {
        const int rb = rfl(ldsi[L::SST + k]), re = rfl(ldsi[L::SST + k + 1]);
        const int Tn = rfl(ldsi[L::STOT + k]);
        const int nitems = (Tn + 63) >> 6;
        const int psv = (lane < re - rb) ? (int)((unsigned)ldsi[L::RECTS + 4 * (rb + min(lane, MAXRS - 1)) + 1] >> 16) : 0x7fffffff;
        int pst16[MAXRS];
#pragma unroll
        for (int rr = 0; rr < MAXRS; ++rr) pst16[rr] = __builtin_amdgcn_readlane(psv, rr);
        for (int it0 = sw; it0 < nitems; it0 += snw * PFD) {
            long long tq1 = 0, tq2 = 0;
            if (ltiming) tq1 = clock64();
#pragma unroll
            for (int j = 0; j < PFD; ++j) {
                const int it = it0 + snw * j;
                Item I = item(it < nitems ? it * 64 + lane : Tn, Tn, rb, pst16);
                if (a.cl) {
#pragma unroll
                    for (int q = 0; q < Q; ++q) pf[j][q] = reinterpret_cast<const f4*>(I.g)[q];
                } else if (!F16) {
#pragma unroll
                    for (int q = 0; q < Q; ++q) {
                        const float* __restrict__ g = I.g + (size_t)(4 * q) * plane;
                        pf[j][q][0] = g[0];
                        pf[j][q][1] = g[plane];
                        pf[j][q][2] = g[2 * plane];
                        pf[j][q][3] = g[3 * plane];
                    }
                }
                pmeta[j] = I.meta;
                pgeo[j] = I.geo;
            }
            if (ltiming) { tq2 = clock64(); lt_issue += tq2 - tq1; }
            write_round();
            if (ltiming) lt_write += clock64() - tq2;
        }
    };

#if D3D_DECOUPLE
#error "the counter hand-off experiment predates the channel-group loop (its counters are per step, not per pass)"
#endif
    if (loader && ring) {
        for (int gi = 0; gi < a.ngroups; ++gi) {
        grp = gi;
        c0 = gi * CH;
        if (FREERUN && ring) {
            stage(0, wave, NWAVES);
            __syncthreads();
            for (int k = 1; k < nsteps; ++k) {
                if (k >= 2) ctr_wait(ldsi + L::CNT + (k - 2), min(SP, nplanes - (k - 2) * SP) * NPIXW);
                stage(k, lw, NLOADW);
                ctr_add(ldsi + L::CNT + MAXSTEPS + k, lane);
            }
        } else if (ring) {
            stage(0, STAGE0_ALL_EFF ? wave : lw, STAGE0_ALL_EFF ? NCOMP + NLOADW : NLOADW);
#if D3D_DECOUPLE
            step_signal(ldsi + L::CNT + 0, lane);
            for (int k = 0; k + 1 < nsteps; ++k) {
                long long tb = 0;
                if (ltiming) tb = clock64();
                if (k > 0) step_wait(ldsi + L::CNT + MAXSTEPS + (k - 1), NCOMP);
                if (ltiming) lt_bar += clock64() - tb;
                stage(k + 1, lw, NLOADW);
                step_signal(ldsi + L::CNT + (k + 1), lane);
            }
#else
            for (int k = 0; k < nsteps; ++k) {
                long long tb = 0;
                if (ltiming) tb = clock64();
                __syncthreads();
                if (ltiming) lt_bar += clock64() - tb;
                if (k + 1 < nsteps) stage(k + 1, lw, NLOADW);
            }
#endif
        }
        __syncthreads();
        }
        if (ltiming && lane == 0) {
            atomicAdd(a.tstats + 2, (unsigned long long)lt_bar);
            atomicAdd(a.tstats + 6, (unsigned long long)lt_issue);
            atomicAdd(a.tstats + 7, (unsigned long long)lt_write);
        }
        return;
    }

    if constexpr (!EARLY_INPUTS) {
        projection_rows();
        lane_inputs();
    } else {
        if (loader) lane_inputs();
    }
    RingView RV[NSRC];
    const int lds0 = lds_base_bytes(lds);
    const float umax = (float)w, vmax = (float)h;
#pragma unroll
    for (int i = 0; i < NSRC; ++i) {
        if (ring && i >= p.n_src) {
            ray[i].rx = 0.0f; ray[i].ry = 0.0f; ray[i].rz = 0.0f;
            T0[i] = -1.0f; T1[i] = -1.0f; T2[i] = 1.0f;
        }
        RV[i].RW = ring ? rfl(ldsi[L::HDR + 4 + 4 * i + 0]) : 1;
        RV[i].RH = ring ? rfl(ldsi[L::HDR + 4 + 4 * i + 1]) : 1;
        RV[i].rowb = ring_row_floats<STRIDE>(RV[i].RW) * 4;
        RV[i].base = lds0 + 4 * (ring ? rfl(ldsi[L::HDR + 4 + 4 * i + 2]) : L::DATA);
#ifdef D3D_RV_VGPR
        asm volatile("" : "+v"(RV[i].RW), "+v"(RV[i].RH), "+v"(RV[i].rowb), "+v"(RV[i].base));
#endif
    }
    const float invV = 1.0f / (float)(p.n_src + 1);
    const size_t cstride_b = (p.plane_major ? plane : (size_t)D * plane) * sizeof(T);
    const size_t cl_step = p.out_cl == 2 ? plane * 16 : 16;

    unsigned long long even_quad = 0;
    auto finalize_store = [&](const f4& s, const f4& qq, unsigned long long& ob, int q) {
        f4 o;
        if (MODE == MODE_VARIANCE) {
            const f2 iv = {invV, invV};
            const f2 ml = lo2(s) * iv, mh = hi2(s) * iv;
            o = cat2(pk_fma(lo2(qq), iv, -(ml * ml)), pk_fma(hi2(qq), iv, -(mh * mh)));
        } else if (MODE == MODE_WEIGHTED) {
            o = s * rden;
        } else {
            o = s;
        }
        if constexpr (OUTCL) {
            if ((q & 1) == 0) {
                even_quad = pack_h16x4(o);
            } else {
                store_sbase_h16x8(ob, pixo, even_quad, pack_h16x4(o));
                ob += cl_step;
            }
        } else {
#pragma unroll
            for (int k = 0; k < 4; ++k) {
                store_sbase(ob, pixb, o[k]);
                ob += cstride_b;
            }
        }
    };
    auto accumulate = [&](f4& s, f4& qq, float& pair_acc, const f4& val, int q, int i) {
        if (MODE == MODE_VARIANCE) {
            const f2 vl = lo2(val), vh = hi2(val);
            s = cat2(lo2(s) + vl, hi2(s) + vh);
            qq = cat2(pk_fma(vl, vl, lo2(qq)), pk_fma(vh, vh, hi2(qq)));
        } else if (MODE == MODE_WEIGHTED) {
#pragma unroll
            for (int k = 0; k < 4; ++k) s[k] = fmaf(val[k] * r[F16 ? 0 : q][k], vw[i], s[k]);
        } else if (MODE == MODE_PAIR) {
#pragma unroll
            for (int k = 0; k < 4; ++k) pair_acc = fmaf(r[F16 ? 0 : q][k], val[k], pair_acc);
        } else {
            s = val;
        }
    };

    const bool timing = D3D_STAMPS && a.tstats != nullptr && wave == 0;
    const bool wtiming = D3D_STAMPS && a.tstats != nullptr;
    long long t_ww = 0;
    long long t_w = 0, t_w0 = 0, t_c = 0, t_mark = 0;
    if (timing) { t_mark = clock64(); if (lane == 0) atomicAdd(a.tstats + 0, (unsigned long long)(t_mark - t_start)); }
#ifdef D3D_YOUNG_PRIO
    if (wave >= NCOMP / 2) __builtin_amdgcn_s_setprio(D3D_YOUNG_PRIO);
#endif
    int kx[NSRC], ky[NSRC];
    int plan_adr = 0;
    auto load_step = [&](int k) {
        if constexpr (VIEW_MAJOR) {
            plan_adr = lds_base_bytes(lds) + 4 * (L::PLAN + (ring ? k : 0) * NSRC * 8);
            return;
        }
#pragma unroll
        for (int i = 0; i < NSRC; ++i) {
            const int* e = ldsi + L::PLAN + ((ring ? k : 0) * NSRC + i) * 8;
            kx[i] = rfl(e[6]);
            ky[i] = rfl(e[7]);
        }
    };
    auto sweep_plane = [&](const int dl_) {
            const int d = ds + dl_;
            float dv;
            if (p.depth_mode == D3D_DEPTH_PER_PIXEL) {
                float t = p.depth[(size_t)d * plane + pix];
                dv = valid ? t : 1.0f;
            } else if (p.depth_mode == D3D_DEPTH_AFFINE) {
                dv = __fadd_rn(aff_lo, __fmul_rn((float)d, aff_step));
            } else {
                dv = lds[L::PMIN + dl_];
            }
            unsigned long long ob = OUTCL ? uniform64(reinterpret_cast<unsigned short*>(p.out) +
                                                      (p.out_cl == 2 ? ((size_t)d * (p.C / 8) + c0 / 8) * plane * 8 : (size_t)d * plane * p.C + c0))
                                          : uniform64(reinterpret_cast<T*>(p.out) + (p.plane_major ? (size_t)d * p.C + c0 : (size_t)c0 * D + d) * plane);
            float pair_acc = 0.0f;
            if (!valid) return;

            if constexpr (VIEW_MAJOR) {
                float sa[Q][CPC], qa[Q][CPC];
#pragma unroll
                for (int q = 0; q < Q; ++q)
#pragma unroll
                    for (int k = 0; k < CPC; ++k) {
                        const float rv = F16 ? rh[F16 ? q : 0][F16 ? k : 0] : r[F16 ? 0 : q][F16 ? 0 : k];
                        sa[q][k] = (MODE == MODE_VARIANCE) ? rv : 0.0f;
                        qa[q][k] = rv * rv;
                    }
                auto accumulate_vm = [&](const float (&val)[CPC], int q, int i) {
#pragma unroll
                    for (int k = 0; k < CPC; k += 2) {
                        const f2 v = {val[k], val[k + 1]};
                        if (MODE == MODE_VARIANCE) {
                            const f2 sn = (f2){sa[q][k], sa[q][k + 1]} + v;
                            const f2 qn = pk_fma(v, v, (f2){qa[q][k], qa[q][k + 1]});
                            sa[q][k] = sn[0]; sa[q][k + 1] = sn[1];
                            qa[q][k] = qn[0]; qa[q][k + 1] = qn[1];
                        } else {
                            sa[q][k] = fmaf(v[0] * r[F16 ? 0 : q][F16 ? 0 : k], vw[i], sa[q][k]);
                            sa[q][k + 1] = fmaf(v[1] * r[F16 ? 0 : q][F16 ? 0 : k + 1], vw[i], sa[q][k + 1]);
                        }
                    }
                };
                if (ring) {
                    const int vt_adr = lds0 + 4 * L::VT;
                    auto geometry = [&](int i) -> TapL {
                        typedef int i4v __attribute__((ext_vector_type(4)));
                        typedef int i2v __attribute__((ext_vector_type(2)));
                        const f4 tv = *(volatile lds_f4_ptr)(unsigned)(vt_adr + 32 * i);
                        const i4v rv = *(volatile __attribute__((address_space(3))) const i4v*)(unsigned)(vt_adr + 32 * i + 16);
                        const i2v kk = *(volatile __attribute__((address_space(3))) const i2v*)(unsigned)(plan_adr + 32 * i + 24);
                        RingView R;
                        R.RW = rv[0]; R.RH = rv[1]; R.rowb = rv[2]; R.base = rv[3];
                        return geo_ring<STRIDE>(ray[i], tv[0], tv[1], tv[2], dv, umax, vmax, kk[0], kk[1], R);
                    };
                    auto fetch = [&](const TapL& g, int q, f4 (&dst)[4]) {
                        dst[0] = lds_read4_abs(g.a0 + q * 16);
                        dst[1] = lds_read4_abs(g.a0 + q * 16 + STRIDE * 4);
                        dst[2] = lds_read4_abs(g.a1 + q * 16);
                        dst[3] = lds_read4_abs(g.a1 + q * 16 + STRIDE * 4);
                    };
                    f4 tp[2][4];
                    TapL gc = geometry(0);
                    fetch(gc, 0, tp[0]);
#pragma unroll
                    for (int i = 0; i < NSRC; ++i) {
                        __builtin_amdgcn_sched_barrier(0);
                        TapL gn = gc;
                        if (i + 1 < NSRC) gn = geometry(i + 1);
#pragma unroll
                        for (int q = 0; q < Q; ++q) {
                            const int u = i * Q + q;
                            if (q + 1 < Q) fetch(gc, q + 1, tp[(u + 1) & 1]);
                            else if (i + 1 < NSRC) fetch(gn, 0, tp[(u + 1) & 1]);
                            f4 (&c)[4] = tp[u & 1];
                            asm volatile("" : "+v"(c[3]));
                            float val[CPC];
                            if constexpr (F16) {
                                const float tw[4] = {gc.nw, gc.ne, gc.sw, gc.se};
#pragma unroll
                                for (int k = 0; k < CPC; ++k) val[k] = 0.0f;
#pragma unroll
                                for (int tp_ = 0; tp_ < 4; ++tp_) {
#pragma unroll
                                    for (int k = 0; k < CPC; k += 2) {
                                        const int wi = k >> 1;
                                        val[k] = fma_mix_lo(c[tp_][wi], tw[tp_], val[k]);
                                        val[k + 1] = fma_mix_hi(c[tp_][wi], tw[tp_], val[k + 1]);
                                    }
                                    if (tp_ < 3) __builtin_amdgcn_sched_barrier(0);
                                }
                            } else {
                                const f4 v4 = blend(c[0], c[1], c[2], c[3], gc.nw, gc.ne, gc.sw, gc.se);
#pragma unroll
                                for (int k = 0; k < CPC; ++k) val[k] = v4[k];
                            }
                            accumulate_vm(val, q, i);
                        }
                        gc = gn;
                    }
                } else {
                    for (int i = 0; i < p.n_src; ++i) {
                        const float* __restrict__ M = p.proj34 + 12 * i;
                        const Ray rr = make_ray(M, xf, yf);
                        float u, v;
                        project(rr, M[3], M[7], M[11], dv, h, w, u, v);
                        const TapG t = make_tap_glb(u, v, h, w);
                        const T* __restrict__ gp = reinterpret_cast<const T*>(p.feats[i + 1]) + (size_t)c0 * plane + t.off;
#pragma unroll
                        for (int q = 0; q < Q; ++q) {
                            float val[CPC];
#pragma unroll
                            for (int k = 0; k < CPC; ++k) {
                                const T* __restrict__ gk = gp + (size_t)(CPC * q + k) * plane;
                                val[k] = fmaf(ldf(gk + t.dyw + t.dx), t.se, fmaf(ldf(gk + t.dyw), t.sw, fmaf(ldf(gk + t.dx), t.ne, ldf(gk) * t.nw)));
                            }
                            accumulate_vm(val, q, i);
                        }
                    }
                }
#pragma unroll
                for (int q = 0; q < Q; ++q)
#pragma unroll
                    for (int k = 0; k < CPC; ++k) {
                        float o;
                        if (MODE == MODE_VARIANCE) {
                            const float m = sa[q][k] * invV;
                            o = fmaf(qa[q][k], invV, -(m * m));
                        } else {
                            o = sa[q][k] * rden;
                        }
                        if constexpr (F16) store_sbase_h(ob, pixb, o);
                        else store_sbase(ob, pixb, o);
                        ob += cstride_b;
                    }
                return;
            }

            if (ring) {
                TapL t[NSRC];
#pragma unroll
                for (int i = 0; i < NSRC; ++i) {
                    t[i] = geo_ring<STRIDE>(ray[i], T0[i], T1[i], T2[i], dv, umax, vmax, kx[i], ky[i], RV[i]);
                }
                constexpr int NU = Q * NSRC;
                constexpr int PD = LDS_PIPE;
                f4 tp[PD + 1][4];
                auto request = [&](int u, f4 (&dst)[4]) {
                    const int q2 = u / NSRC, i2 = u % NSRC;
                    dst[0] = lds_read4_abs(t[i2].a0 + q2 * 16);
                    dst[1] = lds_read4_abs(t[i2].a0 + q2 * 16 + STRIDE * 4);
                    dst[2] = lds_read4_abs(t[i2].a1 + q2 * 16);
                    dst[3] = lds_read4_abs(t[i2].a1 + q2 * 16 + STRIDE * 4);
                };
#pragma unroll
                for (int u = 0; u < PD && u < NU; ++u) request(u, tp[u % (PD + 1)]);
                if (PD == 0) request(0, tp[0]);
                f4 s, qq;
#pragma unroll
                for (int u = 0; u < NU; ++u) {
                    const int q = u / NSRC, i = u % NSRC;
                    if (PD > 0 ? (u + PD < NU) : (u > 0)) request(u + PD, tp[(u + PD) % (PD + 1)]);
                    if (i == 0) {
                        if (MODE == MODE_VARIANCE) { s = r[F16 ? 0 : q]; qq = s * s; }
                        else { s = (f4){0, 0, 0, 0}; qq = s; }
                    }
                    f4 (&c)[4] = tp[u % (PD + 1)];
                    asm volatile("" : "+v"(c[3]));
                    f4 val = blend(c[0], c[1], c[2], c[3], t[i].nw, t[i].ne, t[i].sw, t[i].se);
                    accumulate(s, qq, pair_acc, val, q, i);
                    if (i == NSRC - 1 && MODE != MODE_PAIR) finalize_store(s, qq, ob, q);
                }
            } else {
                TapG t[NSRC];
#pragma unroll
                for (int i = 0; i < NSRC; ++i) {
                    float u, v;
                    project(ray[i], T0[i], T1[i], T2[i], dv, h, w, u, v);
                    t[i] = make_tap_glb(u, v, h, w);
                    if (i >= p.n_src) { t[i].nw = t[i].ne = t[i].sw = t[i].se = 0.0f; t[i].off = 0; t[i].dx = 0; t[i].dyw = 0; }
                }
#pragma unroll
                for (int q = 0; q < Q; ++q) {
                    f4 s, qq;
                    if (MODE == MODE_VARIANCE) { s = r[F16 ? 0 : q]; qq = s * s; }
                    else { s = (f4){0, 0, 0, 0}; qq = s; }
#pragma unroll
                    for (int i = 0; i < NSRC; ++i) {
                        const float* __restrict__ g = p.feats[min(i + 1, p.n_src)] + (size_t)(c0 + 4 * q) * plane + t[i].off;
                        f4 val;
#pragma unroll
                        for (int kk = 0; kk < 4; ++kk) {
                            const float* __restrict__ gk = g + (size_t)kk * plane;
                            val[kk] = fmaf(gk[t[i].dyw + t[i].dx], t[i].se,
                                           fmaf(gk[t[i].dyw], t[i].sw, fmaf(gk[t[i].dx], t[i].ne, gk[0] * t[i].nw)));
                        }
                        accumulate(s, qq, pair_acc, val, q, i);
                    }
                    if (MODE != MODE_PAIR) finalize_store(s, qq, ob, q);
                }
            }
            if (MODE == MODE_PAIR)
                store_sbase(uniform64(p.out + (size_t)d * plane), pixb, pair_acc / (float)CH);
    };
    for (int gi = 0; gi < a.ngroups; ++gi) {
    grp = gi;
    c0 = gi * CH;
    if (gi > 0) load_reference();
    if (FREERUN && ring) {
        stage(0, wave, NWAVES);
        __syncthreads();
        int kcur = 0;
        load_step(0);
        for (;;) {
            int pg = 0;
            if (lane == 0) pg = __hip_atomic_fetch_add(ldsi + L::HDR + 28 + pw, 1, __ATOMIC_RELAXED, __HIP_MEMORY_SCOPE_WORKGROUP);
            pg = rfl(pg);
            if (pg >= nplanes) break;
            if (pg >= (kcur + 1) * SP) {
                while (pg >= (kcur + 1) * SP) ++kcur;
                ctr_wait(ldsi + L::CNT + MAXSTEPS + kcur, NLOADW);
                load_step(kcur);
            }
            sweep_plane(pg);
            ctr_add(ldsi + L::CNT + kcur, lane);
        }
        __syncthreads();
        if (wave == 0) {
            for (int i = lane; i < 2 * MAXSTEPS; i += 64) ldsi[L::CNT + i] = 0;
            if (lane < 2) ldsi[L::HDR + 28 + lane] = 0;
        }
        continue;
    }
    if (!ring) {
        constexpr int NW = NWAVES / NPIXW;
        static_assert(NWAVES % NPIXW == 0, "the loader waves must come in whole sets of pixel waves");
        load_step(0);
        for (int dl_ = wave / NPIXW; dl_ < nplanes; dl_ += NW) sweep_plane(dl_);
        __syncthreads();
        continue;
    }
#if STAGE0_ALL_EFF
    if (ring) stage(0, wave, NCOMP + NLOADW);
#endif
    for (int k = 0; k < nsteps; ++k) {
        if (ring) {
            long long ta = 0;
            if (timing) ta = clock64();
            long long tw0 = 0;
            if (wtiming) tw0 = clock64();
            __syncthreads();
            if (wtiming && k > 0) t_ww += clock64() - tw0;
            if (timing) { t_mark = clock64(); t_w += t_mark - ta; if (k == 0) t_w0 = t_mark - ta; }
        }
        load_step(k);

#if D3D_GRAB
        static_assert(NPIXW <= 2, "one plane counter per step and pixel wave: CNT holds two rows of MAXSTEPS");
        const int spk = min(SP, nplanes - k * SP);
        for (;;) {
            int jg = 0;
            if (lane == 0) jg = __hip_atomic_fetch_add(ldsi + L::CNT + pw * MAXSTEPS + k, 1, __ATOMIC_RELAXED, __HIP_MEMORY_SCOPE_WORKGROUP);
            jg = rfl(jg);
            if (jg >= spk) break;
            const int dl_ = k * SP + jg;
#else
        for (int j = 0; sub + NSUB * j < SP; ++j) {
            const int dl_ = k * SP + sub + NSUB * j;
            if (dl_ >= nplanes) break;
#endif
            sweep_plane(dl_);
        }
        if (timing) t_c += clock64() - t_mark;
        if constexpr (NLOADW == 0) {
            if (ring && k + 1 < nsteps) stage(k + 1, wave, NWAVES);
        }
    }
    __syncthreads();
#if D3D_GRAB
    if (wave == 0) for (int i = lane; i < 2 * MAXSTEPS; i += 64) ldsi[L::CNT + i] = 0;
#endif
    if (timing) t_mark = clock64();
    }
    if (wtiming && lane == 0) atomicAdd(a.tstats + 8 + wave, (unsigned long long)t_ww);
    if (timing && lane == 0) {
        atomicAdd(a.tstats + 1, (unsigned long long)t_w);
        atomicAdd(a.tstats + 5, (unsigned long long)t_w0);
        atomicAdd(a.tstats + 3, (unsigned long long)t_c);
        atomicAdd(a.tstats + 4, (unsigned long long)(clock64() - t_start));
    }
}

struct PackArgs {
    const void* src[D3D_MAX_VIEWS];
};
template <int CH, typename T>
__global__ __launch_bounds__(256) void pack_channel_last_kernel(PackArgs pa, int ngroups, long plane, float* __restrict__ out) {
    constexpr int CW = CH * (int)sizeof(T) / 4, Q = CW / 4, CPC = 16 / (int)sizeof(T);
    const long t = (long)blockIdx.x * 256 + threadIdx.x;
    const long pos = t / Q;
    const int q = (int)(t - pos * Q);
    if (pos >= plane) return;
    const int vg = blockIdx.y;
    const int v = vg / ngroups, g = vg - v * ngroups;
    const T* __restrict__ s = reinterpret_cast<const T*>(pa.src[v]) + ((size_t)g * CH + CPC * q) * plane + pos;
    f4 x;
    if (sizeof(T) == 4) {
        const float* __restrict__ sf = reinterpret_cast<const float*>(s);
        x[0] = sf[0]; x[1] = sf[plane]; x[2] = sf[2 * plane]; x[3] = sf[3 * plane];
    } else {
        const unsigned short* __restrict__ sh = reinterpret_cast<const unsigned short*>(s);
        unsigned wd[4];
#pragma unroll
        for (int k = 0; k < 4; ++k) wd[k] = (unsigned)sh[(2 * k) * plane] | ((unsigned)sh[(2 * k + 1) * plane] << 16);
        x = __builtin_bit_cast(f4, (uint4){wd[0], wd[1], wd[2], wd[3]});
    }
    reinterpret_cast<f4*>(out + ((size_t)vg * plane + pos) * CW)[q] = x;
}

int pack_channel_last_g8(const SweepParams& p, hipStream_t stream) {
    PackArgs pa = {};
    for (int i = 0; i < p.n_src; ++i) pa.src[i] = p.feats[i + 1];
    const long plane = (long)p.h * p.w;
    const int ngroups = p.C / 8;
    hipLaunchKernelGGL((pack_channel_last_kernel<8, float>), dim3((unsigned)ceil_div(plane * 2, 256), p.n_src * ngroups), dim3(256), 0, stream, pa,
                       ngroups, plane, reinterpret_cast<float*>(p.workspace));
    D3D_LAUNCH_CHECK("pack_channel_last_kernel launch (window gather path)");
    return D3D_OK;
}

static int group_channels(int C, int n_src, int elem_bytes);

static void segments(int D, long tiles, int& dseg, int& nseg) {
    int dseg_cap = DSEG_MAX;
#ifdef D3D_EXPERIMENTS
    if (const char* e = getenv("D3D_TILED_DSEG")) dseg_cap = max(NSUB, min(atoi(e), DSEG_MAX));
#endif
    nseg = ceil_div(D, dseg_cap);
    while (tiles * nseg < 4096 && nseg * 2 <= ceil_div(D, 32)) nseg *= 2;
    dseg = ceil_div(D, nseg);
    nseg = ceil_div(D, dseg);
}

#ifndef D3D_CL_MIN_PLANES
#define D3D_CL_MIN_PLANES 96
#endif
static bool wants_channel_last(int D, int elem_bytes) { return elem_bytes == 2 || D >= D3D_CL_MIN_PLANES; }

size_t tiled_workspace_bytes(int n_src, int C, int D, int h, int w, int elem_bytes) {
    if (C % 8 != 0 || n_src > 6 || n_src < 1 || !wants_channel_last(D, elem_bytes)) return 0;
    return (size_t)n_src * C * h * w * elem_bytes;
}

#ifndef D3D_SHALLOW_PLANES
#define D3D_SHALLOW_PLANES 16
#endif
constexpr int SHALLOW_NSUB = 2, SHALLOW_NLOADW = D3D_NLOADW, SHALLOW_NPIXW = 4, SHALLOW_PLANES = D3D_SHALLOW_PLANES;

template <int MODE, int NSRC, int CH, typename T, bool OUTCL = false, bool SHALLOW = false>
static int launch_one(const SweepParams& p, hipStream_t stream) {
    constexpr int CW = CH * (int)sizeof(T) / 4;
    using L = Lds<CW, NSRC>;
    constexpr int LDS_BYTES = 160 * 1024;
    constexpr int NSUBK = SHALLOW ? SHALLOW_NSUB : NSUB, NLOADK = SHALLOW ? SHALLOW_NLOADW : NLOADW;
    constexpr int NPIXK = SHALLOW ? SHALLOW_NPIXW : NPIXW, THK = 2 * NPIXK;
    constexpr int THREADSK = 64 * (NPIXK * NSUBK + NLOADK);
    auto kern = sweep_tiled_kernel<MODE, NSRC, CH, T, OUTCL, NSUBK, NLOADK, NPIXK>;
    if (OUTCL && (size_t)p.h * p.w * p.C * 2 >= ((size_t)1 << 32)) return D3D_ERR_UNSUPPORTED;
    int rc = ensure_dynamic_lds(reinterpret_cast<const void*>(kern), LDS_BYTES);
    if (rc != D3D_OK) return rc;
    TiledArgs a;
    a.ngroups = p.C / CH;
    a.tiles_x = ceil_div(p.w, TW);
    a.tiles_y = ceil_div(p.h, THK);
    a.cap_floats = LDS_BYTES / 4 - L::DATA;
    segments(p.D, (long)a.tiles_x * a.tiles_y * a.ngroups, a.dseg, a.nseg);
    const long nblk = (long)a.tiles_x * a.tiles_y * a.nseg;
    if (nblk > 0x7fffffffL) return D3D_ERR_UNSUPPORTED;
    a.stats = nullptr;
    a.tstats = nullptr;
    a.cl = nullptr;
    {
        bool use_cl = wants_channel_last(p.D, (int)sizeof(T));
#ifdef D3D_EXPERIMENTS
        if (const char* e = getenv("D3D_TILED_CL")) use_cl = atoi(e) != 0;
#endif
        const size_t bytes = (size_t)p.n_src * p.C * p.h * p.w * sizeof(T);
        if (use_cl && p.workspace && p.workspace_bytes >= bytes) {
            PackArgs pa = {};
            for (int i = 0; i < p.n_src; ++i) pa.src[i] = p.feats[i + 1];
            const long plane = (long)p.h * p.w;
            hipLaunchKernelGGL((pack_channel_last_kernel<CH, T>), dim3((unsigned)ceil_div(plane * (CW / 4), 256), p.n_src * a.ngroups),
                               dim3(256), 0, stream, pa, a.ngroups, plane, reinterpret_cast<float*>(p.workspace));
            D3D_LAUNCH_CHECK("pack_channel_last_kernel launch");
            a.cl = reinterpret_cast<const float*>(p.workspace);
        }
        if (sizeof(T) == 2 && !a.cl) return D3D_ERR_UNSUPPORTED;
    }
#ifdef D3D_EXPERIMENTS
    if (getenv("D3D_TILED_STATS")) {
        (void)hipMalloc(&a.stats, 8 * sizeof(unsigned) + 24 * sizeof(unsigned long long));
        (void)hipMemset(a.stats, 0, 8 * sizeof(unsigned) + 24 * sizeof(unsigned long long));
        a.tstats = reinterpret_cast<unsigned long long*>(a.stats + 8);
    }
#endif
    hipLaunchKernelGGL(kern, dim3((unsigned)nblk), dim3(THREADSK), LDS_BYTES, stream, p, a);
    D3D_LAUNCH_CHECK("sweep_tiled_kernel launch");
#ifdef D3D_EXPERIMENTS
    if (a.stats) {
        unsigned hs[8];
        unsigned long long ht[24];
        (void)hipMemcpy(hs, a.stats, sizeof(hs), hipMemcpyDeviceToHost);
        (void)hipMemcpy(ht, a.tstats, sizeof(ht), hipMemcpyDeviceToHost);
        fprintf(stderr, "[d3d tiled timing] per-WG mean cycles: compute wave 0: prologue %.0f | barrier wait %.0f (initial window %.0f) | compute %.0f | total %.0f || loader 0: barrier wait %.0f | decode+issue %.0f | wait+write %.0f\n",
                ht[0] / (double)nblk, ht[1] / (double)nblk, ht[5] / (double)nblk, ht[3] / (double)nblk, ht[4] / (double)nblk,
                ht[2] / (double)nblk, ht[6] / (double)nblk, ht[7] / (double)nblk);
        fprintf(stderr, "[d3d tiled timing] prologue phases: depth range %.0f | candidate windows %.0f | plan tables %.0f (rest: per-lane constants)\n",
                ht[16] / (double)nblk, ht[17] / (double)nblk, ht[18] / (double)nblk);
        fprintf(stderr, "[d3d tiled timing] barrier wait after the first, per compute wave (pixel rows, depth sub-range):");
        for (int wv = 0; wv < NPIXK * NSUBK; ++wv) fprintf(stderr, " %.0f", ht[8 + wv] / (double)nblk);
        fprintf(stderr, "\n");
        fprintf(stderr, "[d3d tiled stats] CH=%d elem=%d wgs=%ld ring=%u fallback=%u mean_step_planes=%.2f mean_steps=%.2f mean_ring_positions=%.0f (cap %d) dseg=%d\n",
                CH, (int)sizeof(T), nblk, hs[0], hs[1], hs[2] / (double)nblk, hs[3] / (double)nblk, hs[0] ? hs[4] / (double)hs[0] : 0.0,
                a.cap_floats / L::STRIDE, a.dseg);
        (void)hipFree(a.stats);
    }
#endif
    return D3D_OK;
}

static int group_channels(int C, int n_src, int elem_bytes) {
    int cg = (n_src > 4 && elem_bytes == 4) ? 8 : (C >= 16 ? 16 : C);
#ifdef D3D_EXPERIMENTS
    if (const char* e = getenv("D3D_TILED_CG")) cg = atoi(e);
#endif
    if (cg != 8 && cg != 16 && cg != 32) cg = 8;
    while (C % cg) cg >>= 1;
    return cg;
}

template <int MODE, int NSRC>
static int launch_ch(const SweepParams& p, hipStream_t stream) {
    const int cg = (MODE == MODE_PAIR) ? p.C : group_channels(p.C, p.n_src, 4);
#ifndef D3D_SHALLOW_CG16
#define D3D_SHALLOW_CG16 0
#endif
    bool shallow = p.D <= SHALLOW_PLANES && (cg == 8 || (D3D_SHALLOW_CG16 && cg == 16));
#ifdef D3D_EXPERIMENTS
    if (const char* e = getenv("D3D_TILED_SHALLOW")) shallow = shallow && atoi(e) != 0;
#endif
    if constexpr (MODE == MODE_VARIANCE) {
        if (p.out_cl) {
            if constexpr (SHALLOW_PLANES > 0) {
                if (shallow && cg == 8) return launch_one<MODE, NSRC, 8, float, true, true>(p, stream);
                if (D3D_SHALLOW_CG16 && shallow && cg == 16) return launch_one<MODE, NSRC, 16, float, true, true>(p, stream);
            }
            switch (cg) {
                case 16: return launch_one<MODE, NSRC, 16, float, true>(p, stream);
                case 8: return launch_one<MODE, NSRC, 8, float, true>(p, stream);
            }
            return D3D_ERR_UNSUPPORTED;
        }
    }
    if (p.out_cl) return D3D_ERR_UNSUPPORTED;
    if constexpr (SHALLOW_PLANES > 0 && (MODE == MODE_VARIANCE || MODE == MODE_WEIGHTED)) {
        if (shallow && cg == 8) return launch_one<MODE, NSRC, 8, float, false, true>(p, stream);
        if (D3D_SHALLOW_CG16 && shallow && cg == 16) return launch_one<MODE, NSRC, 16, float, false, true>(p, stream);
    }
    (void)shallow;
    switch (cg) {
        case 32: return launch_one<MODE, NSRC, 32, float>(p, stream);
        case 16: return launch_one<MODE, NSRC, 16, float>(p, stream);
        case 8: return launch_one<MODE, NSRC, 8, float>(p, stream);
    }
    return D3D_ERR_UNSUPPORTED;
}

template <int NSRC>
static int launch_f16(const SweepParams& p, hipStream_t stream) {
    if (p.C % 16 != 0) return D3D_ERR_UNSUPPORTED;
    return launch_one<MODE_VARIANCE, NSRC, 16, __half>(p, stream);
}

const char* tiled_build_flags() {
    return ""
#ifdef D3D_EXPERIMENTS
           " D3D_EXPERIMENTS"
#endif
#ifdef D3D_DEV_ONLY_HEADLINE
           " D3D_DEV_ONLY_HEADLINE"
#endif
#if D3D_NSUB != 4
           " D3D_NSUB"
#endif
#if D3D_NLOADW != 4
           " D3D_NLOADW"
#endif
#if D3D_LDS_PIPE != 1
           " D3D_LDS_PIPE"
#endif
#if D3D_GRAB
           " D3D_GRAB"
#endif
#if D3D_FREERUN
           " D3D_FREERUN"
#endif
#if D3D_DECOUPLE
           " D3D_DECOUPLE"
#endif
#if STAGE0_ALL != 1
           " STAGE0_ALL"
#endif
#if D3D_SHALLOW_PLANES != 16
           " D3D_SHALLOW_PLANES"
#endif
#if D3D_SHALLOW_CG16
           " D3D_SHALLOW_CG16"
#endif
#if D3D_CL_MIN_PLANES != 96
           " D3D_CL_MIN_PLANES"
#endif
#ifdef D3D_YOUNG_PRIO
           " D3D_YOUNG_PRIO"
#endif
#ifdef D3D_RV_VGPR
           " D3D_RV_VGPR"
#endif
        ;
}

int launch_tiled(int mode, const SweepParams& p, hipStream_t stream) {
#ifdef D3D_DEV_ONLY_HEADLINE
    return launch_one<MODE_VARIANCE, 4, 16, float>(p, stream);
#else
    if (p.C % 8 != 0 || (mode == MODE_PAIR && p.C != 32 && p.C != 16 && p.C != 8)) {
        set_error("tiled kernel unsupported: C=%d", p.C);
        return D3D_ERR_UNSUPPORTED;
    }
    if (p.n_src > 6) {
        set_error("tiled kernel unsupported: %d source views (max 6)", p.n_src);
        return D3D_ERR_UNSUPPORTED;
    }
    if (p.elem_bytes == 2) {
        if (mode != MODE_VARIANCE || p.out_cl) return D3D_ERR_UNSUPPORTED;
        if (p.n_src > 4) return launch_f16<6>(p, stream);
        return p.n_src <= 2 ? launch_f16<2>(p, stream) : launch_f16<4>(p, stream);
    }
    switch (mode) {
        case MODE_VARIANCE:
            if (p.n_src > 4) return launch_ch<MODE_VARIANCE, 6>(p, stream);
            return p.n_src <= 2 ? launch_ch<MODE_VARIANCE, 2>(p, stream) : launch_ch<MODE_VARIANCE, 4>(p, stream);
        case MODE_WEIGHTED:
            if (p.n_src > 4) return launch_ch<MODE_WEIGHTED, 6>(p, stream);
            return p.n_src <= 2 ? launch_ch<MODE_WEIGHTED, 2>(p, stream) : launch_ch<MODE_WEIGHTED, 4>(p, stream);
        case MODE_PAIR: return launch_ch<MODE_PAIR, 1>(p, stream);
        case MODE_WARP: return launch_ch<MODE_WARP, 1>(p, stream);
    }
    set_error("internal: bad mode %d", mode);
    return D3D_ERR_INVALID_ARG;
#endif
}

}
```

include/deep3d_planesweep.h:

```cpp
#ifndef DEEP3D_PLANESWEEP_H
#define DEEP3D_PLANESWEEP_H

#include <stddef.h>
#include <stdint.h>

#ifdef __cplusplus
extern "C" {
#endif

#define D3D_ABI_VERSION 11

#define D3D_OK 0
#define D3D_ERR_INVALID_ARG (-1)
#define D3D_ERR_UNSUPPORTED (-2)
#define D3D_ERR_HIP (-3)

#define D3D_DEPTH_PER_PLANE 0
#define D3D_DEPTH_PER_PIXEL 1
#define D3D_DEPTH_AFFINE 2

#define D3D_MAX_VIEWS 16

typedef void* d3d_stream_t;

int d3d_version(void);

const char* d3d_last_error(void);

int d3d_compose_projections(const float* proj44, int n_views, float* out34, d3d_stream_t stream);

int d3d_debug_force_path(int path);

int d3d_debug_dispatch_counts(unsigned long long* out4, int reset);

const char* d3d_build_flags(void);

const char* d3d_h16_format(void);

size_t d3d_sweep_workspace_bytes(int n_views, int C, int D, int h, int w, int elem_bytes);
size_t d3d_sweep_workspace_bytes_for(int n_views, int C, int D, int h, int w, int elem_bytes, int depth_mode);

int d3d_homo_warp(const float* src, const float* proj34, const float* depth, int depth_mode, int C, int D, int h,
                  int w, float* out, void* workspace, size_t workspace_bytes, d3d_stream_t stream);

int d3d_compose_projections_f64(const double* proj44, int n_views, double* out34, d3d_stream_t stream);
int d3d_homo_warp_f64coord(const float* src, const double* proj34, const float* depth, int depth_mode, int C, int D,
                           int h, int w, float* out, d3d_stream_t stream);

int d3d_variance_volume(const float* const* feats, const float* proj34, const float* depth, int depth_mode,
                        int n_views, int C, int D, int h, int w, float* out, void* workspace, size_t workspace_bytes,
                        d3d_stream_t stream);
int d3d_variance_volume_planes(const float* const* feats, const float* proj34, const float* depth, int depth_mode,
                               int n_views, int C, int D, int h, int w, float* out, void* workspace, size_t workspace_bytes,
                               d3d_stream_t stream);

int d3d_variance_volume_cl_h16(const float* const* feats, const float* proj34, const float* depth, int depth_mode,
                                int n_views, int C, int D, int h, int w, void* out, void* workspace, size_t workspace_bytes,
                                d3d_stream_t stream);
int d3d_variance_volume_cl8_h16(const float* const* feats, const float* proj34, const float* depth, int depth_mode,
                                int n_views, int C, int D, int h, int w, void* out, void* workspace, size_t workspace_bytes,
                                d3d_stream_t stream);

int d3d_variance_volume_f16(const void* const* feats, const float* proj34, const float* depth, int depth_mode,
                            int n_views, int C, int D, int h, int w, void* out, void* workspace,
                            size_t workspace_bytes, d3d_stream_t stream);

int d3d_pair_corr_mean(const float* ref, const float* src, const float* proj34, const float* depth, int depth_mode,
                       int C, int D, int h, int w, float* out, void* workspace, size_t workspace_bytes,
                       d3d_stream_t stream);

int d3d_weighted_corr(const float* const* feats, const float* proj34, const float* weights, const float* depth,
                      int depth_mode, int n_views, int C, int D, int h, int w, int plane_major, float* out, void* workspace,
                      size_t workspace_bytes, d3d_stream_t stream);
int d3d_weighted_corr_cl8_h16(const float* const* feats, const float* proj34, const float* weights, const float* depth,
                              int depth_mode, int n_views, int C, int D, int h, int w, void* out, void* workspace,
                              size_t workspace_bytes, d3d_stream_t stream);


int d3d_softargmin_conf4(const float* cost, const float* depth, int depth_mode, int D, int h, int w,
                         float* depth_out, float* conf_out, d3d_stream_t stream);

int d3d_online_regress_update(const float* reg, const float* dplane, int hd, int wd, int H, int W, float* max_p,
                              float* sum_d, float* sum_p, d3d_stream_t stream);

int d3d_slice_head_regress_h16(const float* up, const float* weight, const float* bias, int transposed, const float* dplane, int hd,
                                int wd, int h, int w, float* max_p, float* sum_d, float* sum_p, d3d_stream_t stream);
int d3d_conv2d_k3_zs_h16_gn(const float* in, int C1, const float* in2, int C2, const void* wpacked, const float* shift, int Co, int H,
                             int W, float* out, double* gn_stats, int gn_split, d3d_stream_t stream);
int d3d_conv2d_k3_wide_h16_gn(const float* in, int C1, const float* in2, int C2, const void* wpacked, const float* shift, int Co, int H,
                               int W, float* out, double* gn_stats, int gn_split, d3d_stream_t stream);
int d3d_convtranspose2d_k3s2_wide_h16(const float* in, const void* wpacked, const float* scale, const float* shift,
                                      const float* skip, int act, int Ci, int Co, int H, int W, float* out, d3d_stream_t stream);
int d3d_conv2d_k3_pair3_bf16x3(const float* img, const float* w0packed, const float* scale0, const float* shift0, int act0,
                               const void* wpacked, const float* scale, const float* shift, int act, int Co, int H, int W,
                               float* out, d3d_stream_t stream);
int d3d_slice_tail_regress_h16(const float* state2, const void* wup_packed, const float* bup, const float* state1, const float* whead,
                                const float* bhead, const float* dplane, int hd, int wd, int h, int w, float* max_p, float* sum_d,
                                float* sum_p, d3d_stream_t stream);
int d3d_slice_tail_regress_same_h16(const float* state2, const void* wup_packed, const float* bup, const float* state1, int skip_after_act,
                                    const float* whead, const float* bhead, const float* dplane, int hd, int wd, int h, int w,
                                    float* max_p, float* sum_d, float* sum_p, d3d_stream_t stream);
int d3d_online_regress_finalize(const float* max_p, const float* sum_d, const float* sum_p, int64_t n,
                                float* depth_out, float* conf_out, d3d_stream_t stream);

int d3d_depth_range_samples(const float* cur_depth, int mode, int D, float interval, int h, int w, float* out,
                            d3d_stream_t stream);

int d3d_resize_bilinear(const float* in, int n, int h, int w, int H, int W, float* out, d3d_stream_t stream);


int d3d_conv3d_k3(const float* in, const float* weight, const float* scale, const float* shift, const float* skip,
                  int relu, int Ci, int Co, int D, int H, int W, int stride, float* out, d3d_stream_t stream);

int d3d_conv3d_k3_co8(const float* in, const float* wpacked, const float* scale, const float* shift, const float* skip,
                      int relu, int Ci, int D, int H, int W, float* out, d3d_stream_t stream);

int d3d_conv3d_k3_c8_h16(const float* in, const void* wpacked, const float* scale, const float* shift, const float* skip,
                          int relu, int Ci, int D, int H, int W, float* out, d3d_stream_t stream);
int d3d_conv3d_k3_zs_h16(const float* in, const void* wpacked, const float* scale, const float* shift, const float* skip,
                          int relu, int Ci, int Co, int D, int H, int W, float* out, d3d_stream_t stream);
int d3d_conv3d_k3_zs_bf16x3(const float* in, const void* wpacked, const float* scale, const float* shift, const float* skip,
                            int relu, int Ci, int Co, int D, int H, int W, float* out, d3d_stream_t stream);
int d3d_conv3d_k3_c1_bf16x3(const float* in, const void* wpacked, const float* scale, const float* shift, const float* skip,
                            int relu, int Ci, int D, int H, int W, float* out, d3d_stream_t stream);


int d3d_convtranspose3d_k3s2_co8(const float* in, const float* wpacked, const float* scale, const float* shift,
                                 const float* skip, int relu, int Ci, int D, int H, int W, float* out,
                                 d3d_stream_t stream);

int d3d_convtranspose3d_k3s2_zs_h16(const float* in, const void* wpacked, const float* scale, const float* shift,
                                     const float* skip, int relu, int Ci, int Co, int D, int H, int W, float* out,
                                     d3d_stream_t stream);
int d3d_convtranspose3d_k3s2_zs_bf16x3(const float* in, const void* wpacked, const float* scale, const float* shift,
                                     const float* skip, int relu, int Ci, int Co, int D, int H, int W, float* out,
                                     d3d_stream_t stream);
int d3d_conv3d_k3s2_zs_bf16x3(const float* in, const void* wpacked, const float* scale, const float* shift, const float* skip,
                              int relu, int Ci, int Co, int D, int H, int W, float* out, d3d_stream_t stream);

int d3d_conv2d_k3_zs_h16(const float* in, int C1, const float* in2, int C2, const void* wpacked, const float* scale,
                          const float* shift, const float* skip, const float* aux1, int act, int ep_split,
                          int skip_after_act, int Co, int H, int W, float* out, d3d_stream_t stream);

int d3d_conv2d_k3_zs_f32(const float* in, int C1, const float* in2, int C2, const void* wpacked, const float* scale,
                         const float* shift, const float* skip, const float* aux1, int act, int ep_split,
                         int skip_after_act, int Co, int H, int W, float* out, d3d_stream_t stream);

int d3d_conv2d_k3_zs_bf16x3(const float* in, int C1, const float* in2, int C2, const void* wpacked, const float* scale,
                            const float* shift, const float* skip, const float* aux1, int act, int ep_split,
                            int skip_after_act, int Co, int H, int W, float* out, d3d_stream_t stream);

int d3d_avgpool2d_4_8(const float* in, int C, int H, int W, float* out4, float* out8, d3d_stream_t stream);
int d3d_conv2d_k1_f32(const float* in, const float* wt, const float* scale, const float* shift, const float* skip, int act,
                      int Ci, int Co, int H, int W, float* out, d3d_stream_t stream);

int d3d_conv3x3_bias_border(float* out, const float* taps, int Co, int H, int W, d3d_stream_t stream);
int d3d_conv1x1_context(const float* f, int Ci, const float* weight, const float* a, int Ha, int Wa, const float* b, int Hb,
                        int Wb, int Co, int H, int W, float* out, d3d_stream_t stream);

int d3d_conv2d_k3s2_zs_h16(const float* in, const void* wpacked, const float* scale, const float* shift, const float* skip,
                            int act, int skip_after_act, int Ci, int Co, int H, int W, float* out, d3d_stream_t stream);
int d3d_conv2d_k3s2_zs_h16_batched(const float* in, const void* wpacked, const float* scale, const float* shift, int act, int Ci, int Co,
                                   int H, int W, int nbatch, int64_t in_bstride, int64_t out_bstride, float* out, d3d_stream_t stream);
int d3d_convtranspose2d_k3s2_zs_h16(const float* in, const void* wpacked, const float* scale, const float* shift,
                                     const float* skip, int act, int skip_after_act, int Ci, int Co, int H, int W, float* out,
                                     d3d_stream_t stream);
int d3d_conv2d_k3s2_zs_f32(const float* in, const void* wpacked, const float* scale, const float* shift, const float* skip,
                           int act, int skip_after_act, int Ci, int Co, int H, int W, float* out, d3d_stream_t stream);
int d3d_convtranspose2d_k3s2_zs_f32(const float* in, const void* wpacked, const float* scale, const float* shift,
                                    const float* skip, int act, int skip_after_act, int Ci, int Co, int H, int W, float* out,
                                    d3d_stream_t stream);
int d3d_conv2d_k3s2_zs_bf16x3(const float* in, const void* wpacked, const float* scale, const float* shift, const float* skip,
                              int act, int skip_after_act, int Ci, int Co, int H, int W, float* out, d3d_stream_t stream);
int d3d_convtranspose2d_k3s2_zs_bf16x3(const float* in, const void* wpacked, const float* scale, const float* shift,
                                       const float* skip, int act, int skip_after_act, int Ci, int Co, int H, int W,
                                       float* out, d3d_stream_t stream);

int d3d_convtranspose2d_k4s2_zs_bf16x3(const float* in, const void* wpacked, const float* scale, const float* shift,
                                       const float* skip, int act, int skip_after_act, int Ci, int Co, int H, int W,
                                       float* out, d3d_stream_t stream);

int d3d_conv2d_k3_wide_h16(const float* in, int C1, const float* in2, int C2, const void* wpacked, const float* scale,
                            const float* shift, const float* skip, int act, int Co, int H, int W, float* out, d3d_stream_t stream);

int d3d_gru_cell_fused_h16(const float* cost, int CP, int HI, int WI, int stride, const float* h, int HID, int H, int W,
                            const void* w1, const void* wg, const float* bg, const void* wc, const float* bc, float* hout,
                            d3d_stream_t stream);
int d3d_gru_cell_fused_cl8_h16(const void* cost_cl8, int CP, const float* h, int HID, int H, int W, const void* w1, const void* wg,
                               const float* bg, const void* wc, const float* bc, float* hout, d3d_stream_t stream);


int d3d_conv2d_k5s2_zs_bf16x3(const float* in, const void* wpacked, const float* scale, const float* shift, const float* skip,
                              int act, int skip_after_act, int Ci, int Co, int H, int W, float* out, d3d_stream_t stream);


int d3d_conv3d_k3_cl_h16(const void* in, int in_cl, const void* wpacked, const float* scale, const float* shift,
                          const void* skip, int relu, int Ci, int Co, int D, int H, int W, void* out, int out_cl,
                          d3d_stream_t stream);
int d3d_conv3d_k3_c1_cl_h16(const void* in, int in_cl, const void* wpacked, const float* scale, const float* shift,
                             const float* skip, int relu, int Ci, int D, int H, int W, float* out, d3d_stream_t stream);
int d3d_conv3d_k3s2_cl_h16(const void* in, const void* wpacked, const float* scale, const float* shift, const void* skip,
                            int relu, int Ci, int Co, int D, int H, int W, void* out, d3d_stream_t stream);
int d3d_convtranspose3d_k3s2_cl_h16(const void* in, const void* wpacked, const float* scale, const float* shift,
                                     const void* skip, int relu, int Ci, int Co, int D, int H, int W, void* out,
                                     int channel_last, d3d_stream_t stream);
int d3d_convtranspose3d_prob_cl_h16(const void* in, const void* wt_folded, const float* scale, const float* shift,
                                     const void* skip, int relu, const void* wprob_kzfolded, const float* prob_bias,
                                     int D, int H, int W, float* out, d3d_stream_t stream);
int d3d_volume_planar_to_cl_h16(const float* in, int C, size_t n, void* out, d3d_stream_t stream);
int d3d_volume_cl_h16_to_planar(const void* in, int C, size_t n, float* out, d3d_stream_t stream);


int d3d_conv2d_k3_stream(const float* in0, int Ci0, const float* in1, int Ci1, const float* wpacked, const float* scale,
                         const float* shift, const float* skip, const float* aux1, int ep_split, int act, int Co, int H,
                         int W, float* out, d3d_stream_t stream);

int d3d_conv1x1_upskip(const float* in, int Ci, const float* wpacked, const float* bias, const float* coarse, int Co, int H,
                       int W, float* out, d3d_stream_t stream);

int d3d_convtranspose3d_k3s2(const float* in, const float* weight, const float* scale, const float* shift,
                             const float* skip, int relu, int Ci, int Co, int D, int H, int W, float* out,
                             d3d_stream_t stream);

int d3d_conv2d_k3(const float* in0, int Ci0, const float* in1, int Ci1, const float* weight, const float* scale,
                  const float* shift, const float* skip, int act, int Co, int H, int W, int stride, float* out,
                  d3d_stream_t stream);

int d3d_convtranspose2d_k3s2(const float* in, const float* weight, const float* scale, const float* shift,
                             const float* skip, int skip_after_act, int act, int Ci, int Co, int H, int W,
                             float* out, d3d_stream_t stream);

int d3d_conv_gemm_f32(const float* in0, int Ci0, const float* in1, int Ci1, const float* wpack, int mpad,
                      const float* scale, const float* shift, const float* skip, int skip_after_act, int act,
                      int Co, int D, int H, int W, int Dg, int Hg, int Wg, int Do, int Ho, int Wo, int istride,
                      int ostride, int oz, int oy, int ox, int ntaps, const signed char* taps_zyx, float* out,
                      d3d_stream_t stream);

int d3d_conv_fold_f32(const float* in0, int Ci0, const float* in1, int Ci1, const float* wpack, int mpad, int M,
                      const float* scale, const float* shift, const float* skip, int skip_after_act, int act,
                      const float* aux1, int ep_split, int Co, int D, int H, int W, int Do, int Ho, int Wo,
                      const int* geom, int ntaps, const signed char* taps_zyx, float* out, d3d_stream_t stream);

int d3d_conv_fold_h16(const float* in0, int Ci0, const float* in1, int Ci1, const float* wpack, int mpad, int M,
                       const float* scale, const float* shift, const float* skip, int skip_after_act, int act,
                       const float* aux1, int ep_split, int Co, int D, int H, int W, int Do, int Ho, int Wo,
                       const int* geom, int ntaps, const signed char* taps_zyx, float* out, d3d_stream_t stream);

int d3d_gru_gates(const float* gates, const float* h, int Hc, int64_t plane, float* rh, float* u,
                  d3d_stream_t stream);
int d3d_gru_update(const float* u, const float* h, const float* convc, int64_t n, float* h_out,
                   d3d_stream_t stream);

int d3d_groupnorm_stats(const float* x, int64_t n, int ngroups, double* stats, d3d_stream_t stream);
int d3d_gru_gates_gn(const float* gates, const double* stats_r, const double* stats_u, const float* gamma_r,
                     const float* beta_r, const float* gamma_u, const float* beta_u, const float* h, int Hc,
                     int64_t plane, float eps, int fast, float* rh, float* u, d3d_stream_t stream);
int d3d_gru_update_gn(const float* o, const double* stats_o, const float* gamma, const float* beta, const float* u,
                      const float* h, int Hc, int64_t plane, float eps, int fast, float* h_out, d3d_stream_t stream);
int d3d_gru_reset_gn(const float* gates, const double* stats_r, const float* gamma_r, const float* beta_r, const float* h, int Hc,
                     int64_t plane, float eps, int fast, float* rh, d3d_stream_t stream);
int d3d_gru_update_gates_gn(const float* o, const double* stats_o, const float* gamma, const float* beta, const float* gates,
                            const double* stats_u, const float* gamma_u, const float* beta_u, const float* h, int Hc, int64_t plane,
                            float eps, int fast, float* h_out, d3d_stream_t stream);
int d3d_gru2_cell_gn_h16(const float* x, int Cx, const float* h, int Hc, int H, int W, const void* wg, const float* bg, const void* wc,
                         const float* bc, const float* gamma_r, const float* beta_r, const float* gamma_u, const float* beta_u,
                         const float* gamma_o, const float* beta_o, float eps, int fast, double* stats_g, double* stats_o, float* gates,
                         float* rh, float* o, float* hout, d3d_stream_t stream);

int d3d_softargmin_conf4_var(const float* cost, const float* depth, int depth_mode, int D, int h, int w, float lamb,
                             float* depth_out, float* conf_out, float* var_out, d3d_stream_t stream);

int d3d_uncertainty_samples(const float* cur_depth, const float* exp_var, int D, int h, int w, float* out,
                            d3d_stream_t stream);

int d3d_pair_softmax_max(const float* score, const float* depth, int depth_mode, int D, int h, int w,
                         float* view_weight, float* pair_depth, d3d_stream_t stream);

#define D3D_FUSION_CAM_DOUBLES 94
int d3d_consistency_check(const float* depth_ref, const float* normal_ref, const float* prob_ref,
                          const float* depth_src, const float* normal_src, const double* cam, int H, int W, int Hs,
                          int Ws, double position_threshold, float depth_threshold, float normal_cos_threshold,
                          float confidence_threshold, unsigned char* mask, float* depth_reprojected,
                          float* depth_src_out, float* xyz_world_src, float* angle_conf, d3d_stream_t stream);
int d3d_fusion_ref_init(const float* depth_ref, const float* normal_ref, const double* cam, int H, int W,
                        float* all_xyz_world, float* conf_sum, int* geo_mask_sum, float* normal_world,
                        d3d_stream_t stream);
int d3d_fusion_accumulate(const float* depth_ref, const float* normal_ref, const float* prob_ref,
                          const float* depth_src, const float* normal_src, const double* cam, int H, int W, int Hs,
                          int Ws, double position_threshold, float depth_threshold, float normal_cos_threshold,
                          float confidence_threshold, int src_idx, int* geo_mask_sum, float* all_xyz_world,
                          float* conf_sum, int* vis, float* depth_src_out, d3d_stream_t stream);
int d3d_fusion_finalize(const float* all_xyz_world, const float* conf_sum, const int* geo_mask_sum, int H, int W,
                        int min_geo_consist_num, float* avg_xyz_world, unsigned char* final_mask, d3d_stream_t stream);

size_t d3d_fusion_points_scratch_bytes(int H, int W);
int d3d_fusion_mark_points(const float* avg_xyz_world, const unsigned char* final_mask, int H, int W, int skip_line,
                           const double* scene_range_xy, void* scratch, unsigned char* keep, unsigned* counts,
                           d3d_stream_t stream);
int d3d_fusion_gather_points(const float* avg_xyz_world, const unsigned char* keep, const int* const* vis, int n_vis,
                             const float* color, const float* normal_world, int H, int W, void* scratch, float* out_xyz,
                             int* out_color, float* out_normal, int* out_views, int* out_nviews, d3d_stream_t stream);


int d3d_flip_rows(const float* const* maps, int n, int H, int W, float* out, d3d_stream_t stream);

int d3d_center_image_u8(const unsigned char* img, int h, int w, int channels, int y0, int x0, int H, int W, int mode,
                        unsigned long long* sums, float* out, d3d_stream_t stream);

int d3d_normals_from_depth(const float* depth, const float* kinv, int B, int H, int W, int nei, float* normal,
                           float* encoded, d3d_stream_t stream);

size_t d3d_dsm_scratch_bytes(long long n_points, int W, int H, int select);
int d3d_dsm_from_points(const float* xyz, long long n_points, double x_min, double y_max, double unit_x, double unit_y,
                        double z_min, double z_max, int W, int H, int select, double trim, int min_points, void* scratch,
                        size_t scratch_bytes, float* height, int* count, d3d_stream_t stream);

int d3d_dsm_fill_moving_average(const float* in, float* out, int W, int H, int radius, d3d_stream_t stream);

size_t d3d_dsm_mesh_scratch_bytes(long long n_faces, int W, int H);
int d3d_dsm_from_mesh(const float* vertices, long long n_vertices, const int* faces, long long n_faces, double x_min, double y_max,
                      double unit_x, double unit_y, double z_min, double z_max, int W, int H, void* scratch, size_t scratch_bytes,
                      float* height, d3d_stream_t stream);

typedef struct d3d_ortho_view {
    double R[9];
    double t[3];
    double K[9];
    double C[3];
    const float* depth;
    const unsigned int* rgba;
    int W, H;
    int id;
    int pad;
} d3d_ortho_view_t;

size_t d3d_ortho_scratch_bytes(int W, int H, int n_views);
int d3d_ortho_select(const float* height, double x_min, double y_max, double unit_x, double unit_y, int W, int H,
                     const d3d_ortho_view_t* views, int n_views, double depth_tolerance, void* scratch, size_t scratch_bytes,
                     long long* key, d3d_stream_t stream);

int d3d_ortho_colorize(const float* height, double x_min, double y_max, double unit_x, double unit_y, int W, int H,
                       const long long* key, const d3d_ortho_view_t* views, int n_views, unsigned int* rgba, int* view_out,
                       d3d_stream_t stream);

typedef struct d3d_mesh_grid {
    double x_min, y_min, z_min, voxel;
    int nx, ny, nz;
    int bx, by, bz;
} d3d_mesh_grid_t;

typedef struct d3d_mesh_view {
    double R[9];
    double t[3];
    double K[9];
    const float* depth;
    const float* conf;
    int W, H;
} d3d_mesh_view_t;

size_t d3d_mesh_scan_scratch_bytes(long long n);

int d3d_mesh_mark(const d3d_mesh_grid_t* grid, const d3d_mesh_view_t* views, int n_views, int max_pixels, double conf_threshold,
                  unsigned char* marks, d3d_stream_t stream);

int d3d_mesh_bricks(const d3d_mesh_grid_t* grid, const unsigned char* marks, void* scratch, size_t scratch_bytes, int* brick_index,
                    int* brick_list, long long* n_bricks, d3d_stream_t stream);

int d3d_mesh_integrate(const d3d_mesh_grid_t* grid, const int* brick_list, int n_bricks, const d3d_mesh_view_t* views, int n_views,
                       double trunc, double conf_threshold, float* sum, int* count, d3d_stream_t stream);

int d3d_mesh_count(const d3d_mesh_grid_t* grid, const int* brick_list, const int* brick_index, int n_bricks, const float* sum,
                   const int* count, int min_views, void* scratch, size_t scratch_bytes, unsigned char* edges, int* vert_base,
                   int* face_base, long long* totals, d3d_stream_t stream);

int d3d_mesh_emit(const d3d_mesh_grid_t* grid, const int* brick_list, const int* brick_index, int n_bricks, const float* sum,
                  const int* count, int min_views, const unsigned char* edges, const int* vert_base, const int* face_base,
                  float* vertices, int* faces, int* referenced, d3d_stream_t stream);

int d3d_mesh_compact(const float* vertices, long long n_vertices, int* faces, long long n_faces, const int* referenced, void* scratch,
                     size_t scratch_bytes, int* remap, float* out_vertices, long long* n_kept, d3d_stream_t stream);

size_t d3d_mesh_adjacency_scratch_bytes(long long n_vertices, long long n_faces);

int d3d_mesh_adjacency(const int* faces, long long n_faces, long long n_vertices, void* scratch, size_t scratch_bytes, long long* offset,
                       int* nbr, unsigned char* fixed, d3d_stream_t stream);

int d3d_mesh_components(const int* faces, long long n_faces, long long n_vertices, int* label, int* flag, int* rounds, d3d_stream_t stream);

size_t d3d_mesh_stats_scratch_bytes(long long n_vertices);

int d3d_mesh_component_stats(const float* vertices, long long n_vertices, const int* faces, long long n_faces, const int* label,
                             void* scratch, size_t scratch_bytes, int* face_count, float* box, double* diag, float* global_box,
                             double* global_diag, d3d_stream_t stream);

size_t d3d_mesh_filter_scratch_bytes(long long n_faces);

int d3d_mesh_filter(const int* faces, long long n_faces, long long n_vertices, const int* label, const int* face_count, const double* diag,
                    const double* global_diag, long long min_faces, double spurious, void* scratch, size_t scratch_bytes, int* out_faces,
                    int* referenced, long long* n_kept, d3d_stream_t stream);

int d3d_mesh_smooth(const float* vertices, long long n_vertices, const long long* offset, const int* nbr, const unsigned char* fixed,
                    float lambda, int iterations, float* work, float* out, d3d_stream_t stream);

size_t d3d_mesh_decimate_incidence_scratch_bytes(long long n_vertices, long long n_faces);

int d3d_mesh_decimate_incidence(const int* faces, long long n_faces, long long n_vertices, void* scratch, size_t scratch_bytes,
                                int* face_offset, int* face_index, d3d_stream_t stream);

int d3d_mesh_decimate_quadrics(const float* vertices, long long n_vertices, const int* faces, long long n_faces, const int* face_offset,
                               const int* face_index, double* quadric, d3d_stream_t stream);

size_t d3d_mesh_decimate_edges_scratch_bytes(long long n_vertices);

int d3d_mesh_decimate_edges(const long long* offset, const int* nbr, long long n_vertices, void* scratch, size_t scratch_bytes,
                            long long max_edges, int* edges, long long* n_edges, d3d_stream_t stream);

int d3d_mesh_decimate_candidates(const float* vertices, long long n_vertices, const int* faces, long long n_faces, const long long* offset,
                                 const int* nbr, const unsigned char* fixed, const int* face_offset, const int* face_index,
                                 const double* quadric, const int* edges, const long long* n_edges, long long max_edges, float* target,
                                 float* cost, long long* key, d3d_stream_t stream);

size_t d3d_mesh_decimate_select_scratch_bytes(void);

int d3d_mesh_decimate_select(const long long* key, long long max_edges, long long k, void* scratch, size_t scratch_bytes,
                             long long* threshold, d3d_stream_t stream);

int d3d_mesh_decimate_claim(const long long* offset, const int* nbr, long long n_vertices, const int* edges, const long long* key,
                            const long long* n_edges, long long max_edges, const long long* threshold, long long* claim,
                            long long* n_winners, d3d_stream_t stream);

int d3d_mesh_decimate_apply(const float* vertices, long long n_vertices, const long long* offset, const int* nbr, const unsigned char* fixed,
                            const int* edges, const long long* key, const float* target, const long long* n_edges, long long max_edges,
                            const long long* threshold, const long long* claim, float* out_vertices, int* remap, unsigned char* win,
                            long long* n_winners, d3d_stream_t stream);

size_t d3d_mesh_decimate_faces_scratch_bytes(long long n_faces);

int d3d_mesh_decimate_faces(const int* faces, long long n_faces, long long n_vertices, const int* remap, void* scratch, size_t scratch_bytes,
                            int* out_faces, int* referenced, long long* n_kept, d3d_stream_t stream);

#define D3D_MESH_HOLE_MAX_EDGES 1024

size_t d3d_mesh_holes_scratch_bytes(long long n_vertices);

int d3d_mesh_boundary(const int* faces, long long n_faces, long long n_vertices, const int* face_offset, const int* face_index,
                      int* out_count, int* in_count, int* successor, int* owner, unsigned char* boundary, d3d_stream_t stream);

int d3d_mesh_boundary_loops(const int* faces, long long n_faces, long long n_vertices, const unsigned char* boundary, const int* out_count,
                            const int* in_count, int* label, int* count, int* bad, int* flag, int* rounds, d3d_stream_t stream);

int d3d_mesh_holes_plan(const float* vertices, long long n_vertices, const int* faces, long long n_faces, const int* successor,
                        const int* owner, const int* label, const int* count, const int* bad, int max_edges, void* scratch,
                        size_t scratch_bytes, double* s, float* centroid, int* qualify, int* position, int* vertex_offset, int* face_offset,
                        long long* totals, d3d_stream_t stream);

int d3d_mesh_holes_emit(const float* vertices, long long n_vertices, const int* faces, long long n_faces, const int* successor,
                        const int* label, const int* qualify, const int* position, const int* vertex_offset, const int* face_offset,
                        const float* centroid, long long n_holes, long long n_added, float* out_vertices, int* out_faces,
                        d3d_stream_t stream);

size_t d3d_texture_scratch_bytes(long long n_faces, int n_views);

int d3d_texture_select(const float* vertices, long long n_vertices, const int* faces, long long n_faces, const d3d_ortho_view_t* views,
                       int n_views, double depth_tolerance, void* scratch, size_t scratch_bytes, long long* key, d3d_stream_t stream);

int d3d_texture_edges(const int* faces, long long n_faces, long long n_vertices, const long long* key, long long* edge_key,
                      d3d_stream_t stream);

int d3d_texture_charts(const long long* edge_sorted, const int* face_sorted, long long n_pairs, const long long* key, long long n_faces,
                       void* scratch, size_t scratch_bytes, int* label, int* chart, int* flag, long long* n_charts, int* rounds,
                       d3d_stream_t stream);

int d3d_texture_rects(const float* vertices, long long n_vertices, const int* faces, long long n_faces, const long long* key,
                      const int* chart, long long n_charts, const d3d_ortho_view_t* cams, int n_cams, int pad, int* rect,
                      d3d_stream_t stream);

int d3d_texture_fill(const int* work, long long n_work, const int* table, long long n_charts, const long long* page_row, int n_pages,
                     const d3d_ortho_view_t* views, int n_views, int page_width, unsigned int* atlas, d3d_stream_t stream);

int d3d_texture_empty(unsigned int* atlas, long long n_texels, unsigned int empty_rgba, d3d_stream_t stream);

int d3d_texture_texcoords(const float* vertices, long long n_vertices, const int* faces, long long n_faces, const long long* key,
                          const int* chart, const int* table, long long n_charts, const long long* page_row, int n_pages,
                          const d3d_ortho_view_t* cams, int n_cams, int page_width, float* texcoord, int* texnumber,
                          d3d_stream_t stream);

#ifdef __cplusplus
}
#endif
#endif
```

Before: 20980 Mvoxels/s.

## Make tiled sweep kernel persistent with per-XCD work queues and plan-ahead

Replaces the one-workgroup-per-tile launch with a persistent grid capped at the CU count. Each workgroup pulls tile/depth-segment items from per-XCD atomic queues held in the workspace. Loader waves can plan the next item's depth range, candidate windows and plan tables into a global slot while the current item computes, so the per-item prologue overlaps with compute. This adds atomics, extra barriers, workspace space and more complex control flow, and dynamic scheduling may change cache locality and load balance.

```diff
diff --git a/deep3d_aerial_amd/_lib.py b/deep3d_aerial_amd/_lib.py
--- a/deep3d_aerial_amd/_lib.py
+++ b/deep3d_aerial_amd/_lib.py
@@ -22,6 +22,8 @@
     "d3d_compose_projections": [_vp, _i, _vp, _vp],
     "d3d_debug_force_path": [_i],
     "d3d_debug_dispatch_counts": [_vp, _i],
+    "d3d_debug_tiled_grid": [_i],
+    "d3d_debug_tiled_queue_offset": ([_i, _i, _i, _i, _i, _i], _sz),
     "d3d_build_flags": ([], ctypes.c_char_p),
     "d3d_h16_format": ([], ctypes.c_char_p),
     "d3d_compose_projections_f64": [_vp, _i, _vp, _vp],
diff --git a/deep3d_aerial_amd/csrc/planesweep.hip b/deep3d_aerial_amd/csrc/planesweep.hip
--- a/deep3d_aerial_amd/csrc/planesweep.hip
+++ b/deep3d_aerial_amd/csrc/planesweep.hip
@@ -49,6 +49,8 @@
 int launch_tiled(int mode, const struct SweepParams& p, hipStream_t stream);
 int launch_window(int mode, const struct SweepParams& p, hipStream_t stream, bool forced);
 size_t tiled_workspace_bytes(int n_src, int C, int D, int h, int w, int elem_bytes);
+size_t tiled_queue_offset(int n_src, int C, int D, int h, int w, int elem_bytes);
+void set_tiled_grid_cap(int max_workgroups);
 size_t window_workspace_bytes(int n_src, int C, int D, int h, int w, int elem_bytes);
 const char* tiled_build_flags();
 const char* window_build_flags();
@@ -377,6 +379,16 @@
     return D3D_OK;
 }
 
+int d3d_debug_tiled_grid(int max_workgroups) {
+    D3D_REQUIRE(max_workgroups >= 0, "max_workgroups must be >= 0 (0: no cap)");
+    set_tiled_grid_cap(max_workgroups);
+    return D3D_OK;
+}
+
+size_t d3d_debug_tiled_queue_offset(int n_views, int C, int D, int h, int w, int elem_bytes) {
+    return tiled_queue_offset(n_views - 1, C, D, h, w, elem_bytes);
+}
+
 size_t d3d_sweep_workspace_bytes_for(int n_views, int C, int D, int h, int w, int elem_bytes, int depth_mode) {
     if (n_views < 2 || C <= 0 || D <= 0 || h <= 1 || w <= 1 || (elem_bytes != 4 && elem_bytes != 2)) return 0;
     const size_t a = tiled_workspace_bytes(n_views - 1, C, D, h, w, elem_bytes);
diff --git a/deep3d_aerial_amd/csrc/planesweep_tiled.hip b/deep3d_aerial_amd/csrc/planesweep_tiled.hip
--- a/deep3d_aerial_amd/csrc/planesweep_tiled.hip
+++ b/deep3d_aerial_amd/csrc/planesweep_tiled.hip
@@ -5,6 +5,7 @@
 #include "sweep_params.h"
 #include "sweep_device.h"
 
+#include <atomic>
 #include <cstdlib>
 
 namespace d3d {
@@ -64,7 +65,15 @@
     const float* cl;
     unsigned long long* tstats;
     unsigned* stats;
+    int* queue;
+    int* slots;
+    int nitems;
 };
+
+constexpr int QUEUE_INTS = 16;
+constexpr int SLOT_INTS = 12288;
+constexpr int MAX_PERSISTENT_WGS = 256;
+constexpr int PLAN_PHASES = 6;
 
 template <int CW, int NSRC>
 struct Lds {
@@ -203,7 +212,6 @@
     extern __shared__ __attribute__((aligned(16))) float lds[];
     int* ldsi = reinterpret_cast<int*>(lds);
 
-    const long long t_start = D3D_CLOCK();
     const int tid = threadIdx.x;
     const int lane = tid & 63;
     const int wave = rfl(tid >> 6);
@@ -214,20 +222,59 @@
     const int h = p.h, w = p.w, D = p.D;
     const size_t plane = (size_t)h * w;
 
-    int b = blockIdx.x;
-    {
+    struct Geo {
+        int x0, y0, x1c, y1c;
+        int ds, nplanes;
+    };
+    auto decode_item = [&](int b) __attribute__((always_inline)) -> Geo {
+        const int ty = b % a.tiles_y;
+        const int seg = (b / a.tiles_y) % a.nseg;
+        const int tx = b / (a.tiles_y * a.nseg);
+        Geo g;
+        g.x0 = tx * TW; g.y0 = ty * TH;
+        g.x1c = min(g.x0 + TW - 1, w - 1); g.y1c = min(g.y0 + TH - 1, h - 1);
+        g.ds = seg * a.dseg;
+        g.nplanes = min(g.ds + a.dseg, D) - g.ds;
+        return g;
+    };
+    const bool persistent = a.queue != nullptr;
+    auto take_item = [&]() __attribute__((always_inline)) -> int {
+        const int xcd = blockIdx.x & 7;
+        for (int j = 0; j < 8; ++j) {
+            const int x = (xcd + j) & 7;
+            const int beg = (int)((long long)a.nitems * x / 8), len = (int)((long long)a.nitems * (x + 1) / 8) - beg;
+            if (__hip_atomic_load(a.queue + x, __ATOMIC_RELAXED, __HIP_MEMORY_SCOPE_AGENT) >= len) continue;
+            const int i = __hip_atomic_fetch_add(a.queue + x, 1, __ATOMIC_RELAXED, __HIP_MEMORY_SCOPE_AGENT);
+            if (i < len) return beg + i;
+        }
+        return -1;
+    };
+    constexpr int CT = L::DATA;
+    constexpr int CHD = CT + NCAND * NSRC * 64 * 4;
+    static_assert(CHD + NCAND * NSRC * 4 <= SLOT_INTS, "plan slot too small");
+    int* const slot = persistent ? a.slots + (size_t)blockIdx.x * SLOT_INTS : nullptr;
+    constexpr int NEXT = L::HDR + 31, TAKEN = L::HDR + 30;
+
+    int cur = blockIdx.x;
+    if (!persistent) {
         const int nblk = gridDim.x;
         const int per = nblk / 8;
-        if (nblk % 8 == 0) b = (b % 8) * per + b / 8;
-    }
-    const int ty = b % a.tiles_y;
-    const int seg = (b / a.tiles_y) % a.nseg;
-    const int tx = b / (a.tiles_y * a.nseg);
-    const int x0 = tx * TW, y0 = ty * TH;
-    const int ds = seg * a.dseg;
-    const int de = min(ds + a.dseg, D);
-    const int nplanes = de - ds;
-    const int x1c = min(x0 + TW - 1, w - 1), y1c = min(y0 + TH - 1, h - 1);
+        if (nblk % 8 == 0) cur = (cur % 8) * per + cur / 8;
+    }
+    bool planned = false;
+    for (;;) {
+    if (persistent && !planned) {
+        __syncthreads();
+        if (tid == 0) ldsi[TAKEN] = take_item();
+        __syncthreads();
+        cur = rfl(ldsi[TAKEN]);
+    }
+    if (cur < 0) break;
+    const long long t_start = D3D_CLOCK();
+    const Geo G = decode_item(cur);
+    const int x0 = G.x0, y0 = G.y0;
+    const int ds = G.ds;
+    const int nplanes = G.nplanes;
 
     const int l5 = lane & 31;
     const int pxl = (l5 < 4) ? l5 : (l5 < 12) ? l5 + 4 : (l5 < 20) ? l5 - 8 : (l5 < 28) ? l5 - 20 : l5 - 16;
@@ -243,7 +290,7 @@
     int grp = 0, c0 = 0;
     Ray ray[NSRC];
     float T0[NSRC], T1[NSRC], T2[NSRC];
-    auto projection_rows = [&]() {
+    auto projection_rows = [&]() __attribute__((always_inline)) {
 #pragma unroll
         for (int i = 0; i < NSRC; ++i) {
             const float* __restrict__ M = p.proj34 + 12 * min(i, p.n_src - 1);
@@ -255,7 +302,7 @@
     if constexpr (EARLY_INPUTS) projection_rows();
     f4 r[F16 ? 1 : Q];
     float rh[F16 ? Q : 1][8];
-    auto load_reference = [&]() {
+    auto load_reference = [&]() __attribute__((always_inline)) {
         if (F16) {
 #pragma unroll
             for (int q = 0; q < Q; ++q)
@@ -277,7 +324,7 @@
     float vw[NSRC];
     float rden = 0.0f;
     float aff_lo = 1.0f, aff_step = 0.0f;
-    auto lane_inputs = [&]() {
+    auto lane_inputs = [&]() __attribute__((always_inline)) {
         if (MODE == MODE_WEIGHTED) {
             float den = 1e-5f;
 #pragma unroll
@@ -297,11 +344,13 @@
     if (EARLY_INPUTS && !loader) lane_inputs();
 
     for (int i = tid; i < 2 * STRIDE; i += THREADS) lds[L::ZERO + i] = 0.0f;
+    auto depth_range = [&](float* Tf, const Geo& g, int t, int nt, int wv, int nwv) __attribute__((always_inline)) {
+    const int x0 = g.x0, y0 = g.y0, ds = g.ds, nplanes = g.nplanes;
     if (p.depth_mode == D3D_DEPTH_PER_PLANE) {
-        for (int i = tid; i < nplanes; i += THREADS) {
+        for (int i = t; i < nplanes; i += nt) {
             float dv = p.depth[ds + i];
-            lds[L::PMIN + i] = dv;
-            lds[L::PMAX + i] = dv;
+            Tf[L::PMIN + i] = dv;
+            Tf[L::PMAX + i] = dv;
         }
     } else if (p.depth_mode == D3D_DEPTH_AFFINE) {
         float blo[(TW * TH) / 64], bst[(TW * TH) / 64];
@@ -315,7 +364,7 @@
             blo[k] = p.depth[qi];
             bst[k] = p.depth[plane + qi];
         }
-        for (int i = wave; i < nplanes; i += NWAVES) {
+        for (int i = wv; i < nplanes; i += nwv) {
             float lo = INFINITY, hi = -INFINITY;
 #pragma unroll
             for (int k = 0; k < (TW * TH) / 64; ++k) {
@@ -325,12 +374,12 @@
             lo = wave_min(lo);
             hi = wave_max(hi);
             if (lane == 0) {
-                lds[L::PMIN + i] = lo;
-                lds[L::PMAX + i] = hi;
+                Tf[L::PMIN + i] = lo;
+                Tf[L::PMAX + i] = hi;
             }
         }
     } else {
-        for (int i = wave; i < nplanes; i += NWAVES) {
+        for (int i = wv; i < nplanes; i += nwv) {
             float lo = INFINITY, hi = -INFINITY;
 #pragma unroll
             for (int k = 0; k < (TW * TH) / 64; ++k) {
@@ -345,19 +394,20 @@
             lo = wave_min(lo);
             hi = wave_max(hi);
             if (lane == 0) {
-                lds[L::PMIN + i] = lo;
-                lds[L::PMAX + i] = hi;
-            }
-        }
-    }
+                Tf[L::PMIN + i] = lo;
+                Tf[L::PMAX + i] = hi;
+            }
+        }
+    }
+    };
+    if (!planned) depth_range(lds, G, tid, THREADS, wave, NWAVES);
     __syncthreads();
     const long long t_range = D3D_CLOCK();
 
-    constexpr int CT = L::DATA;
-    constexpr int CHD = CT + NCAND * NSRC * 64 * 4;
-    auto cand_planes = [](int c) { return c < 3 ? NSUB * (4 >> c) : max(NSUB / 2, 1); };
-    auto candidate_windows = [&](int cand, int vsel) {
+    auto cand_planes = [](int c) __attribute__((always_inline)) { return c < 3 ? NSUB * (4 >> c) : max(NSUB / 2, 1); };
+    auto candidate_windows = [&](int* Ti, float* Tf, const Geo& g, int cand, int vsel) __attribute__((always_inline)) {
         {
+            const int x0 = g.x0, y0 = g.y0, x1c = g.x1c, y1c = g.y1c, nplanes = g.nplanes;
             const int SPc = cand_planes(cand);
             const int nstepc = (nplanes + SPc - 1) / SPc;
             const bool feasible = nstepc <= MAXSTEPS;
@@ -365,8 +415,8 @@
             const int p0 = min(lane * SPc, nplanes - 1), p1 = min(lane * SPc + SPc, nplanes);
             float lo = INFINITY, hi = -INFINITY;
             for (int i = p0; i < p1; ++i) {
-                lo = fminf(lo, lds[L::PMIN + i]);
-                hi = fmaxf(hi, lds[L::PMAX + i]);
+                lo = fminf(lo, Tf[L::PMIN + i]);
+                hi = fmaxf(hi, Tf[L::PMAX + i]);
             }
             const float* __restrict__ M = p.proj34 + 12 * min(vsel, p.n_src - 1);
             float umin = INFINITY, umax = -INFINITY, vmin = INFINITY, vmax = -INFINITY;
@@ -405,29 +455,26 @@
             }
             const int RWc = max(wave_maxi(ux), 1), RHc = max(wave_maxi(uy), 1);
             const int badc = (__any(!ok) || !feasible) ? 1 : 0;
-            int* e = ldsi + CT + ((cand * NSRC + vsel) * 64 + lane) * 4;
+            int* e = Ti + CT + ((cand * NSRC + vsel) * 64 + lane) * 4;
             e[0] = wx0; e[1] = wy0; e[2] = ww; e[3] = wh;
             if (lane == 0) {
-                int* hd = ldsi + CHD + (cand * NSRC + vsel) * 4;
+                int* hd = Ti + CHD + (cand * NSRC + vsel) * 4;
                 hd[0] = RWc; hd[1] = RHc; hd[2] = badc; hd[3] = nstepc;
             }
         }
     };
-    constexpr int NCAND1 = NCAND - 1;
-    for (int wk = wave; wk < NCAND1 * NSRC; wk += NWAVES) candidate_windows(wk / NSRC, wk % NSRC);
-    __syncthreads();
-    const long long t_p1 = D3D_CLOCK();
-    auto plan_tables = [&](int cbeg, int cend) {
+    auto plan_tables = [&](int* Ti, float* Tf, const Geo& g, int cbeg, int cend) __attribute__((always_inline)) {
+        const int nplanes = g.nplanes;
         int mode = 0, sp_sel = NSUB, nsteps_sel = (nplanes + NSUB - 1) / NSUB;
         for (int cand = cbeg; cand < cend && !mode; ++cand) {
-            const int nsteps = ldsi[CHD + (cand * NSRC) * 4 + 3];
+            const int nsteps = Ti[CHD + (cand * NSRC) * 4 + 3];
             const bool act = lane < nsteps;
             int wx0[NSRC], wy0[NSRC], ww[NSRC], wh[NSRC], RW[NSRC], RH[NSRC];
             int bad = 0, total = 0, totalq = 0;
             int RWq[NSRC], RHq[NSRC];
 #pragma unroll
             for (int i = 0; i < NSRC; ++i) {
-                const int* hd = ldsi + CHD + (cand * NSRC + i) * 4;
+                const int* hd = Ti + CHD + (cand * NSRC + i) * 4;
                 RW[i] = hd[0]; RH[i] = hd[1]; bad |= hd[2];
                 RWq[i] = (RW[i] + RING_RW_QUANT - 1) / RING_RW_QUANT * RING_RW_QUANT;
                 RHq[i] = (RH[i] + RING_RH_QUANT - 1) / RING_RH_QUANT * RING_RH_QUANT;
@@ -442,7 +489,7 @@
             if (bad || total > a.cap_floats) continue;
 #pragma unroll
             for (int i = 0; i < NSRC; ++i) {
-                const int* e = ldsi + CT + ((cand * NSRC + i) * 64 + lane) * 4;
+                const int* e = Ti + CT + ((cand * NSRC + i) * 64 + lane) * 4;
                 wx0[i] = e[0]; wy0[i] = e[1]; ww[i] = e[2]; wh[i] = e[3];
             }
             if (!bad && total <= a.cap_floats) {
@@ -460,7 +507,7 @@
                     basev[i] = base;
                     dims_ok = dims_ok && RW[i] < 256 && RH[i] < 256;
                     if (act) {
-                        int* e = ldsi + L::PLAN + (lane * NSRC + i) * 8;
+                        int* e = Ti + L::PLAN + (lane * NSRC + i) * 8;
                         e[0] = wx0[i]; e[1] = wy0[i]; e[2] = ww[i]; e[3] = wh[i];
                         e[4] = oxv[i];
                         e[5] = oyv[i];
@@ -468,21 +515,21 @@
                         e[7] = oyv[i] - wy0[i];
                     }
                     if (lane == 0) {
-                        ldsi[L::HDR + 4 + 4 * i + 0] = RW[i];
-                        ldsi[L::HDR + 4 + 4 * i + 1] = RH[i];
-                        ldsi[L::HDR + 4 + 4 * i + 2] = base;
-                        ldsi[L::HDR + 4 + 4 * i + 3] = RW[i] | (RH[i] << 8) | ((base >> 2) << 16);
+                        Ti[L::HDR + 4 + 4 * i + 0] = RW[i];
+                        Ti[L::HDR + 4 + 4 * i + 1] = RH[i];
+                        Ti[L::HDR + 4 + 4 * i + 2] = base;
+                        Ti[L::HDR + 4 + 4 * i + 3] = RW[i] | (RH[i] << 8) | ((base >> 2) << 16);
                         if constexpr (VIEW_MAJOR) {
                             const float* __restrict__ M = p.proj34 + 12 * min(i, p.n_src - 1);
                             const bool dummy = i >= p.n_src;
-                            lds[L::VT + 8 * i + 0] = dummy ? -1.0f : M[3];
-                            lds[L::VT + 8 * i + 1] = dummy ? -1.0f : M[7];
-                            lds[L::VT + 8 * i + 2] = dummy ? 1.0f : M[11];
-                            lds[L::VT + 8 * i + 3] = 0.0f;
-                            ldsi[L::VT + 8 * i + 4] = RW[i];
-                            ldsi[L::VT + 8 * i + 5] = RH[i];
-                            ldsi[L::VT + 8 * i + 6] = ring_row_floats<STRIDE>(RW[i]) * 4;
-                            ldsi[L::VT + 8 * i + 7] = lds_base_bytes(lds) + 4 * base;
+                            Tf[L::VT + 8 * i + 0] = dummy ? -1.0f : M[3];
+                            Tf[L::VT + 8 * i + 1] = dummy ? -1.0f : M[7];
+                            Tf[L::VT + 8 * i + 2] = dummy ? 1.0f : M[11];
+                            Tf[L::VT + 8 * i + 3] = 0.0f;
+                            Ti[L::VT + 8 * i + 4] = RW[i];
+                            Ti[L::VT + 8 * i + 5] = RH[i];
+                            Ti[L::VT + 8 * i + 6] = ring_row_floats<STRIDE>(RW[i]) * 4;
+                            Ti[L::VT + 8 * i + 7] = lds_base_bytes(lds) + 4 * base;
                         }
                     }
                     base += ring_row_floats<STRIDE>(RW[i]) * (RH[i] + 1);
@@ -525,15 +572,15 @@
                     mode = 0;
                 } else {
                     int idx = incl - nrect;
-                    if (act) ldsi[L::SST + lane] = idx;
-                    if (lane == nsteps - 1) ldsi[L::SST + nsteps] = incl;
+                    if (act) Ti[L::SST + lane] = idx;
+                    if (lane == nsteps - 1) Ti[L::SST + nsteps] = incl;
                     int pstart = 0;
 #pragma unroll
                     for (int i = 0; i < NSRC; ++i)
 #pragma unroll
                         for (int r = 0; r < 4; ++r)
                             if (cnt[i][r] > 0) {
-                                int* e = ldsi + L::RECTS + 4 * idx;
+                                int* e = Ti + L::RECTS + 4 * idx;
                                 e[0] = (rx[i][r] + 1) | ((ry[i][r] + 1) << 16);
                                 e[1] = rwid[i][r] | (i << 12) | (pstart << 16);
                                 e[2] = nel[i][r];
@@ -541,25 +588,38 @@
                                 pstart += nel[i][r];
                                 ++idx;
                             }
-                    if (act) ldsi[L::STOT + lane] = pstart;
+                    if (act) Ti[L::STOT + lane] = pstart;
                 }
             }
         }
         if (lane == 0) {
-            ldsi[L::HDR + 0] = mode;
-            ldsi[L::HDR + 1] = sp_sel;
-            ldsi[L::HDR + 2] = nsteps_sel;
-        }
-        for (int i = lane; i < 2 * MAXSTEPS; i += 64) ldsi[L::CNT + i] = 0;
-        if (lane < 2) ldsi[L::HDR + 28 + lane] = 0;
-    };
-    if (wave == 0) plan_tables(0, NCAND1);
-    __syncthreads();
-    if (rfl(ldsi[L::HDR + 0]) == 0) {
+            Ti[L::HDR + 0] = mode;
+            Ti[L::HDR + 1] = sp_sel;
+            Ti[L::HDR + 2] = nsteps_sel;
+        }
+        for (int i = lane; i < 2 * MAXSTEPS; i += 64) Ti[L::CNT + i] = 0;
+        if (lane < 2) Ti[L::HDR + 28 + lane] = 0;
+    };
+    constexpr int NCAND1 = NCAND - 1;
+    long long t_p1 = t_range;
+    if (!planned) {
+        for (int wk = wave; wk < NCAND1 * NSRC; wk += NWAVES) candidate_windows(ldsi, lds, G, wk / NSRC, wk % NSRC);
         __syncthreads();
-        for (int wk = wave; wk < NSRC; wk += NWAVES) candidate_windows(NCAND1, wk);
+        t_p1 = D3D_CLOCK();
+        if (wave == 0) plan_tables(ldsi, lds, G, 0, NCAND1);
         __syncthreads();
-        if (wave == 0) plan_tables(NCAND1, NCAND);
+        if (rfl(ldsi[L::HDR + 0]) == 0) {
+            __syncthreads();
+            for (int wk = wave; wk < NSRC; wk += NWAVES) candidate_windows(ldsi, lds, G, NCAND1, wk);
+            __syncthreads();
+            if (wave == 0) plan_tables(ldsi, lds, G, NCAND1, NCAND);
+            __syncthreads();
+        }
+    } else {
+        typedef int i4c __attribute__((ext_vector_type(4)));
+        static_assert(L::PMIN % 4 == 0 && L::DATA % 4 == 0 && L::HDR % 4 == 0, "tables are copied in 16-byte pieces");
+        for (int i = L::PMIN / 4 + tid; i < L::DATA / 4; i += THREADS)
+            if (i != (L::HDR + 28) / 4) reinterpret_cast<i4c*>(ldsi)[i] = reinterpret_cast<const i4c*>(slot)[i];
         __syncthreads();
     }
     if (D3D_STAMPS && a.tstats && tid == 0) {
@@ -571,6 +631,7 @@
     const int ring = rfl(ldsi[L::HDR + 0]);
     const int SP = rfl(ldsi[L::HDR + 1]);
     const int nsteps = rfl(ldsi[L::HDR + 2]);
+    if (persistent && tid == 0) atomicAdd(a.queue + (ring ? 8 : 9), 1);
     if (D3D_STAMPS && a.stats && tid == 0) {
         atomicAdd(a.stats + (ring ? 0 : 1), 1u);
         atomicAdd(a.stats + 2, (unsigned)SP);
@@ -593,7 +654,7 @@
         const long long di = reinterpret_cast<long long>(p.feats[i + 1]);
         fdelta[i] = (i < p.n_src) ? di - d0 : 0;
     }
-    auto item = [&](int el, int Tn, int rb, const int (&pst16)[MAXRS]) -> Item {
+    auto item = [&](int el, int Tn, int rb, const int (&pst16)[MAXRS]) __attribute__((always_inline)) -> Item {
         Item I;
         const bool live = el < Tn;
         int ridx = rb - 1;
@@ -627,7 +688,7 @@
         I.geo = e7 & 0xffff;
         return I;
     };
-    auto put = [&](int meta, int geo, int q, f4 v) {
+    auto put = [&](int meta, int geo, int q, f4 v) __attribute__((always_inline)) {
         if (meta >= 0) {
             const int dst = (meta & 0xfffff) + 4 * q;
             const int RWv = geo & 0xff, RHv = geo >> 8;
@@ -642,15 +703,15 @@
     };
     f4 pf[PFD][Q];
     int pmeta[PFD], pgeo[PFD];
-    auto write_round = [&]() {
+    auto write_round = [&]() __attribute__((always_inline)) {
 #pragma unroll
         for (int j = 0; j < PFD; ++j)
 #pragma unroll
             for (int q = 0; q < Q; ++q) put(pmeta[j], pgeo[j], q, pf[j][q]);
     };
     const bool ltiming = D3D_STAMPS && a.tstats != nullptr && lw == 0;
-    long long lt_desc = 0, lt_issue = 0, lt_write = 0, lt_bar = 0;
-    auto stage = [&](int k, int sw, int snw) {
+    long long lt_desc = 0, lt_issue = 0, lt_write = 0, lt_bar = 0, lt_plan = 0;
+    auto stage = [&](int k, int sw, int snw) __attribute__((always_inline)) {
         const int rb = rfl(ldsi[L::SST + k]), re = rfl(ldsi[L::SST + k + 1]);
         const int Tn = rfl(ldsi[L::STOT + k]);
         const int nitems = (Tn + 63) >> 6;
@@ -690,6 +751,36 @@
 #if D3D_DECOUPLE
 #error "the counter hand-off experiment predates the channel-group loop (its counters are per step, not per pass)"
 #endif
+    const bool plan_ahead = persistent && ring && !FREERUN && !D3D_DECOUPLE && NLOADW > 0;
+    auto plan_phase = [&](int ph) __attribute__((always_inline)) {
+        int* const Ti = slot;
+        float* const Tf = reinterpret_cast<float*>(slot);
+        if (ph == 0) {
+            if (lw == 0) {
+                int n = 0;
+                if (lane == 0) n = take_item();
+                n = rfl(n);
+                if (lane == 0) ldsi[NEXT] = n;
+            }
+            return;
+        }
+        const int nxt = rfl(ldsi[NEXT]);
+        if (nxt < 0) return;
+        const Geo g = decode_item(nxt);
+        if (ph == 1) {
+            depth_range(Tf, g, lw * 64 + lane, NLOADW * 64, lw, NLOADW);
+        } else if (ph == 2) {
+            for (int wk = lw; wk < NCAND1 * NSRC; wk += NLOADW) candidate_windows(Ti, Tf, g, wk / NSRC, wk % NSRC);
+        } else if (ph == 3) {
+            if (lw == 0) plan_tables(Ti, Tf, g, 0, NCAND1);
+        } else if (rfl(__hip_atomic_load(Ti + L::HDR + 0, __ATOMIC_RELAXED, __HIP_MEMORY_SCOPE_WORKGROUP)) == 0) {
+            if (ph == 4) {
+                for (int wk = lw; wk < NSRC; wk += NLOADW) candidate_windows(Ti, Tf, g, NCAND1, wk);
+            } else if (lw == 0) {
+                plan_tables(Ti, Tf, g, NCAND1, NCAND);
+            }
+        }
+    };
     if (loader && ring) {
         for (int gi = 0; gi < a.ngroups; ++gi) {
         grp = gi;
@@ -715,12 +806,19 @@
                 step_signal(ldsi + L::CNT + (k + 1), lane);
             }
 #else
-            for (int k = 0; k < nsteps; ++k) {
+            const int nbar = plan_ahead && gi == a.ngroups - 1 ? max(nsteps, PLAN_PHASES) : nsteps;
+            for (int k = 0; k < nbar; ++k) {
                 long long tb = 0;
                 if (ltiming) tb = clock64();
                 __syncthreads();
                 if (ltiming) lt_bar += clock64() - tb;
                 if (k + 1 < nsteps) stage(k + 1, lw, NLOADW);
+                if (plan_ahead && gi == a.ngroups - 1 && k >= nbar - PLAN_PHASES) {
+                    long long tp = 0;
+                    if (ltiming) tp = clock64();
+                    plan_phase(k - (nbar - PLAN_PHASES));
+                    if (ltiming) lt_plan += clock64() - tp;
+                }
             }
 #endif
         }
@@ -730,9 +828,9 @@
             atomicAdd(a.tstats + 2, (unsigned long long)lt_bar);
             atomicAdd(a.tstats + 6, (unsigned long long)lt_issue);
             atomicAdd(a.tstats + 7, (unsigned long long)lt_write);
-        }
-        return;
-    }
+            atomicAdd(a.tstats + 19, (unsigned long long)lt_plan);
+        }
+    } else {
 
     if constexpr (!EARLY_INPUTS) {
         projection_rows();
@@ -762,7 +860,7 @@
     const size_t cl_step = p.out_cl == 2 ? plane * 16 : 16;
 
     unsigned long long even_quad = 0;
-    auto finalize_store = [&](const f4& s, const f4& qq, unsigned long long& ob, int q) {
+    auto finalize_store = [&](const f4& s, const f4& qq, unsigned long long& ob, int q) __attribute__((always_inline)) {
         f4 o;
         if (MODE == MODE_VARIANCE) {
             const f2 iv = {invV, invV};
@@ -788,7 +886,7 @@
             }
         }
     };
-    auto accumulate = [&](f4& s, f4& qq, float& pair_acc, const f4& val, int q, int i) {
+    auto accumulate = [&](f4& s, f4& qq, float& pair_acc, const f4& val, int q, int i) __attribute__((always_inline)) {
         if (MODE == MODE_VARIANCE) {
             const f2 vl = lo2(val), vh = hi2(val);
             s = cat2(lo2(s) + vl, hi2(s) + vh);
@@ -814,7 +912,7 @@
 #endif
     int kx[NSRC], ky[NSRC];
     int plan_adr = 0;
-    auto load_step = [&](int k) {
+    auto load_step = [&](int k) __attribute__((always_inline)) {
         if constexpr (VIEW_MAJOR) {
             plan_adr = lds_base_bytes(lds) + 4 * (L::PLAN + (ring ? k : 0) * NSRC * 8);
             return;
@@ -826,7 +924,7 @@
             ky[i] = rfl(e[7]);
         }
     };
-    auto sweep_plane = [&](const int dl_) {
+    auto sweep_plane = [&](const int dl_) __attribute__((always_inline)) {
             const int d = ds + dl_;
             float dv;
             if (p.depth_mode == D3D_DEPTH_PER_PIXEL) {
@@ -853,7 +951,7 @@
                         sa[q][k] = (MODE == MODE_VARIANCE) ? rv : 0.0f;
                         qa[q][k] = rv * rv;
                     }
-                auto accumulate_vm = [&](const float (&val)[CPC], int q, int i) {
+                auto accumulate_vm = [&](const float (&val)[CPC], int q, int i) __attribute__((always_inline)) {
 #pragma unroll
                     for (int k = 0; k < CPC; k += 2) {
                         const f2 v = {val[k], val[k + 1]};
@@ -870,7 +968,7 @@
                 };
                 if (ring) {
                     const int vt_adr = lds0 + 4 * L::VT;
-                    auto geometry = [&](int i) -> TapL {
+                    auto geometry = [&](int i) __attribute__((always_inline)) -> TapL {
                         typedef int i4v __attribute__((ext_vector_type(4)));
                         typedef int i2v __attribute__((ext_vector_type(2)));
                         const f4 tv = *(volatile lds_f4_ptr)(unsigned)(vt_adr + 32 * i);
@@ -880,7 +978,7 @@
                         R.RW = rv[0]; R.RH = rv[1]; R.rowb = rv[2]; R.base = rv[3];
                         return geo_ring<STRIDE>(ray[i], tv[0], tv[1], tv[2], dv, umax, vmax, kk[0], kk[1], R);
                     };
-                    auto fetch = [&](const TapL& g, int q, f4 (&dst)[4]) {
+                    auto fetch = [&](const TapL& g, int q, f4 (&dst)[4]) __attribute__((always_inline)) {
                         dst[0] = lds_read4_abs(g.a0 + q * 16);
                         dst[1] = lds_read4_abs(g.a0 + q * 16 + STRIDE * 4);
                         dst[2] = lds_read4_abs(g.a1 + q * 16);
@@ -972,7 +1070,7 @@
                 constexpr int NU = Q * NSRC;
                 constexpr int PD = LDS_PIPE;
                 f4 tp[PD + 1][4];
-                auto request = [&](int u, f4 (&dst)[4]) {
+                auto request = [&](int u, f4 (&dst)[4]) __attribute__((always_inline)) {
                     const int q2 = u / NSRC, i2 = u % NSRC;
                     dst[0] = lds_read4_abs(t[i2].a0 + q2 * 16);
                     dst[1] = lds_read4_abs(t[i2].a0 + q2 * 16 + STRIDE * 4);
@@ -1102,6 +1200,8 @@
             if (ring && k + 1 < nsteps) stage(k + 1, wave, NWAVES);
         }
     }
+    if (plan_ahead && gi == a.ngroups - 1)
+        for (int k = nsteps; k < PLAN_PHASES; ++k) __syncthreads();
     __syncthreads();
 #if D3D_GRAB
     if (wave == 0) for (int i = lane; i < 2 * MAXSTEPS; i += 64) ldsi[L::CNT + i] = 0;
@@ -1114,6 +1214,12 @@
         atomicAdd(a.tstats + 5, (unsigned long long)t_w0);
         atomicAdd(a.tstats + 3, (unsigned long long)t_c);
         atomicAdd(a.tstats + 4, (unsigned long long)(clock64() - t_start));
+    }
+    }
+    if (D3D_STAMPS && a.tstats && tid == 0) atomicAdd(a.tstats + 20, (unsigned long long)(clock64() - t_start));
+    if (!persistent) break;
+    planned = plan_ahead;
+    if (planned) cur = rfl(ldsi[NEXT]);
     }
 }
 
@@ -1173,9 +1279,32 @@
 #endif
 static bool wants_channel_last(int D, int elem_bytes) { return elem_bytes == 2 || D >= D3D_CL_MIN_PLANES; }
 
+static size_t channel_last_bytes(int n_src, int C, int D, int h, int w, int elem_bytes) {
+    return wants_channel_last(D, elem_bytes) ? (size_t)n_src * C * h * w * elem_bytes : 0;
+}
+size_t tiled_queue_offset(int n_src, int C, int D, int h, int w, int elem_bytes) {
+    return (channel_last_bytes(n_src, C, D, h, w, elem_bytes) + 255) & ~(size_t)255;
+}
 size_t tiled_workspace_bytes(int n_src, int C, int D, int h, int w, int elem_bytes) {
-    if (C % 8 != 0 || n_src > 6 || n_src < 1 || !wants_channel_last(D, elem_bytes)) return 0;
-    return (size_t)n_src * C * h * w * elem_bytes;
+    if (C % 8 != 0 || n_src > 6 || n_src < 1) return 0;
+    const long items = (long)ceil_div(w, TW) * ceil_div(h, TH) * ceil_div(D, 32);
+    const long nwg = items < MAX_PERSISTENT_WGS ? items : MAX_PERSISTENT_WGS;
+    return tiled_queue_offset(n_src, C, D, h, w, elem_bytes) + (size_t)QUEUE_INTS * 4 + (size_t)nwg * SLOT_INTS * 4;
+}
+
+static std::atomic<int> g_grid_cap{0};
+void set_tiled_grid_cap(int max_workgroups) { g_grid_cap.store(max_workgroups, std::memory_order_relaxed); }
+
+static int compute_units() {
+    static std::atomic<int> cus[16];
+    int dev = 0;
+    if (hipGetDevice(&dev) != hipSuccess) return MAX_PERSISTENT_WGS;
+    int n = (dev >= 0 && dev < 16) ? cus[dev].load(std::memory_order_relaxed) : 0;
+    if (n <= 0) {
+        if (hipDeviceGetAttribute(&n, hipDeviceAttributeMultiprocessorCount, dev) != hipSuccess || n <= 0) n = MAX_PERSISTENT_WGS;
+        if (dev >= 0 && dev < 16) cus[dev].store(n, std::memory_order_relaxed);
+    }
+    return n;
 }
 
 #ifndef D3D_SHALLOW_PLANES
@@ -1230,7 +1359,30 @@
         a.tstats = reinterpret_cast<unsigned long long*>(a.stats + 8);
     }
 #endif
-    hipLaunchKernelGGL(kern, dim3((unsigned)nblk), dim3(THREADSK), LDS_BYTES, stream, p, a);
+    a.queue = nullptr;
+    a.slots = nullptr;
+    a.nitems = (int)nblk;
+    long grid = nblk;
+    if (!SHALLOW && !D3D_FREERUN && !D3D_DECOUPLE && NLOADK > 0 && p.workspace) {
+        bool on = true;
+#ifdef D3D_EXPERIMENTS
+        if (const char* e = getenv("D3D_TILED_PERSISTENT")) on = atoi(e) != 0;
+#endif
+        long nwg = min((long)min(compute_units(), MAX_PERSISTENT_WGS), nblk);
+        const int cap = g_grid_cap.load(std::memory_order_relaxed);
+        if (cap > 0) nwg = min(nwg, (long)cap);
+        const size_t off = tiled_queue_offset(p.n_src, p.C, p.D, p.h, p.w, (int)sizeof(T));
+        if (on && p.workspace_bytes >= off + (size_t)QUEUE_INTS * 4 + (size_t)nwg * SLOT_INTS * 4) {
+            a.queue = reinterpret_cast<int*>(reinterpret_cast<char*>(p.workspace) + off);
+            a.slots = a.queue + QUEUE_INTS;
+            grid = nwg;
+            if (hipMemsetAsync(a.queue, 0, QUEUE_INTS * sizeof(int), stream) != hipSuccess) {
+                set_error("sweep_tiled_kernel: clearing the item queue failed");
+                return D3D_ERR_HIP;
+            }
+        }
+    }
+    hipLaunchKernelGGL(kern, dim3((unsigned)grid), dim3(THREADSK), LDS_BYTES, stream, p, a);
     D3D_LAUNCH_CHECK("sweep_tiled_kernel launch");
 #ifdef D3D_EXPERIMENTS
     if (a.stats) {
@@ -1243,6 +1395,8 @@
                 ht[2] / (double)nblk, ht[6] / (double)nblk, ht[7] / (double)nblk);
         fprintf(stderr, "[d3d tiled timing] prologue phases: depth range %.0f | candidate windows %.0f | plan tables %.0f (rest: per-lane constants)\n",
                 ht[16] / (double)nblk, ht[17] / (double)nblk, ht[18] / (double)nblk);
+        fprintf(stderr, "[d3d tiled timing] grid %ld workgroups (%s) | loader 0: planning the next item %.0f | item, start to end %.0f (x items / workgroups = a workgroup's busy cycles)\n",
+                grid, a.queue ? "persistent" : "one item each", ht[19] / (double)nblk, ht[20] / (double)nblk);
         fprintf(stderr, "[d3d tiled timing] barrier wait after the first, per compute wave (pixel rows, depth sub-range):");
         for (int wv = 0; wv < NPIXK * NSUBK; ++wv) fprintf(stderr, " %.0f", ht[8 + wv] / (double)nblk);
         fprintf(stderr, "\n");
diff --git a/include/deep3d_planesweep.h b/include/deep3d_planesweep.h
--- a/include/deep3d_planesweep.h
+++ b/include/deep3d_planesweep.h
@@ -32,6 +32,10 @@
 int d3d_debug_force_path(int path);
 
 int d3d_debug_dispatch_counts(unsigned long long* out4, int reset);
+
+int d3d_debug_tiled_grid(int max_workgroups);
+
+size_t d3d_debug_tiled_queue_offset(int n_views, int C, int D, int h, int w, int elem_bytes);
 
 const char* d3d_build_flags(void);
 
```

Result: slower. 19830 Mvoxels/s (-5.5%).
